# DanEngelbrecht/longtail

Measured on AMD Instinct MI355X. Metric: ingest GB/s (chunk+hash+compress), higher is better.
Workload: dtype u8/u32

## Files before the change

### include/longtail_hip.h

```cpp
#ifndef LONGTAIL_HIP_H
#define LONGTAIL_HIP_H

#include "longtail_abi.h"

#if defined(_WIN32)
#define LTHIP_EXPORT
#else
#define LTHIP_EXPORT __attribute__((visibility("default")))
#endif

#ifdef __cplusplus
extern "C" {
#endif


LTHIP_EXPORT struct Longtail_ChunkerAPI* Longtail_CreateHipChunkerAPI(void);

LTHIP_EXPORT struct Longtail_HashAPI* Longtail_CreateHipBlake3HashAPI(void);

LTHIP_EXPORT struct Longtail_HashAPI* Longtail_CreateHipBlake2HashAPI(void);

LTHIP_EXPORT struct Longtail_HashAPI* Longtail_CreateHipMeowHashAPI(void);

LTHIP_EXPORT struct Longtail_CompressionAPI* Longtail_CreateHipLZ4CompressionAPI(void);
LTHIP_EXPORT struct Longtail_CompressionAPI* Longtail_CompressionRegistry_CreateForHipLZ4(uint32_t compression_type, uint32_t* out_settings);
LTHIP_EXPORT uint32_t Longtail_GetHipLZ4DefaultQuality(void);

LTHIP_EXPORT struct Longtail_CompressionAPI* Longtail_CreateHipZStdCompressionAPI(void);
LTHIP_EXPORT struct Longtail_CompressionAPI* Longtail_CompressionRegistry_CreateForHipZstd(uint32_t compression_type, uint32_t* out_settings);

typedef void* (*Longtail_Hip_AllocFunc)(const char* context, size_t size);
typedef void (*Longtail_Hip_FreeFunc)(void* p);
LTHIP_EXPORT void Longtail_Hip_SetAllocator(Longtail_Hip_AllocFunc alloc_func, Longtail_Hip_FreeFunc free_func);

LTHIP_EXPORT int Longtail_Hip_SetDevice(int device);
LTHIP_EXPORT int Longtail_Hip_SetBlockingWaits(int on);
LTHIP_EXPORT int lthip_set_blocking_waits(int device, int on);

LTHIP_EXPORT int Longtail_Hip_GetLastError(void);

LTHIP_EXPORT uint64_t Longtail_Hip_PinnedBytes(void);
LTHIP_EXPORT void Longtail_Hip_BatchStats(uint64_t* out_batches, uint64_t* out_windows);
LTHIP_EXPORT void Longtail_Hip_CodecBatchStats(uint64_t* out_submissions, uint64_t* out_blocks);
LTHIP_EXPORT void Longtail_Hip_MemoStats(uint64_t* out_puts, uint64_t* out_hits);


typedef struct lthip_ctx lthip_ctx;
typedef struct lthip_plan lthip_plan;

#define LTHIP_STREAM_PRIVATE ((void*)(intptr_t)-1)
LTHIP_EXPORT int lthip_ctx_create(int device, void* hip_stream, lthip_ctx** out_ctx);
LTHIP_EXPORT void lthip_ctx_destroy(lthip_ctx* ctx);
LTHIP_EXPORT int lthip_ctx_sync(lthip_ctx* ctx);
LTHIP_EXPORT const char* lthip_ctx_error(const lthip_ctx* ctx);
LTHIP_EXPORT int lthip_device_count(void);
LTHIP_EXPORT const char* lthip_build_id(void);
#define LTHIP_ABI_VERSION 3
LTHIP_EXPORT int lthip_abi_version(void);

LTHIP_EXPORT int lthip_malloc_device(lthip_ctx* ctx, size_t bytes, void** out);
LTHIP_EXPORT void lthip_free_device(lthip_ctx* ctx, void* p);
LTHIP_EXPORT int lthip_malloc_pinned(lthip_ctx* ctx, size_t bytes, void** out);
LTHIP_EXPORT void lthip_free_pinned(lthip_ctx* ctx, void* p);
LTHIP_EXPORT int lthip_copy_h2d(lthip_ctx* ctx, void* d_dst, const void* h_src, size_t bytes);
LTHIP_EXPORT int lthip_copy_d2h(lthip_ctx* ctx, void* h_dst, const void* d_src, size_t bytes);
LTHIP_EXPORT int lthip_link_copy(lthip_ctx* ctx, void* dst, const void* src, size_t bytes);

enum lthip_kernel_id
{
    LTHIP_K_BUZHASH = 0,
    LTHIP_K_SELECT = 1,
    LTHIP_K_COMPACT = 2,
    LTHIP_K_B3_LEAF = 3,
    LTHIP_K_B3_PARENT = 4,
    LTHIP_K_LZ4_SEG = 5,
    LTHIP_K_LZ4_STITCH = 6,
    LTHIP_K_OTHER = 7,
    LTHIP_K_ZSTD_ENC = 8,
    LTHIP_K_GATHER = 9,
    LTHIP_K_BLAKE2S = 10,
    LTHIP_K_COUNT = 11
};
LTHIP_EXPORT int lthip_timing_enable(lthip_ctx* ctx, int on);
LTHIP_EXPORT int lthip_timing_reset(lthip_ctx* ctx);
LTHIP_EXPORT int lthip_timing_get(lthip_ctx* ctx, int kernel_id, double* out_total_ms, uint64_t* out_launches);

LTHIP_EXPORT int lthip_plan_create(lthip_ctx* ctx, uint32_t part_count, const uint64_t* part_offsets ,
                                   const uint64_t* part_sizes , uint32_t min_chunk, uint32_t avg_chunk,
                                   uint32_t max_chunk, lthip_plan** out_plan);
LTHIP_EXPORT int lthip_plan_resize_single(lthip_ctx* ctx, lthip_plan* plan, uint64_t size);
LTHIP_EXPORT int lthip_plan_reaim(lthip_ctx* ctx, lthip_plan* plan, uint32_t part_count, const uint64_t* part_offsets ,
                                  const uint64_t* part_sizes );
LTHIP_EXPORT void lthip_plan_destroy(lthip_ctx* ctx, lthip_plan* plan);
LTHIP_EXPORT uint64_t lthip_plan_chunk_capacity(const lthip_plan* plan);
LTHIP_EXPORT uint32_t lthip_plan_slices(const lthip_plan* plan);

LTHIP_EXPORT int lthip_chunk_hash(lthip_ctx* ctx, const lthip_plan* plan, const void* d_data, uint64_t* d_chunk_offsets,
                                  uint32_t* d_chunk_lens, uint64_t* d_chunk_hashes, uint32_t* d_part_first,
                                  uint64_t* out_total);

LTHIP_EXPORT int lthip_chunk_from_buffer(lthip_ctx* ctx, const void* d_data, uint64_t size, uint32_t min_chunk,
                                         uint32_t avg_chunk, uint32_t max_chunk, uint64_t* out_len);

LTHIP_EXPORT int lthip_divtest_eval(uint32_t discriminator, uint32_t hash);

LTHIP_EXPORT int lthip_hash_ranges(lthip_ctx* ctx, const void* d_data, uint64_t range_count, const uint64_t* d_offsets,
                                   const uint32_t* d_lens, uint32_t max_len ,
                                   uint64_t* d_hashes);

LTHIP_EXPORT int lthip_hash_one(lthip_ctx* ctx, const void* in, uint32_t len, uint64_t* out);

#define LTHIP_B3_STREAM_BATCH (1u << 20)
#define LTHIP_B3_STREAM_STACK_BYTES 2048u
LTHIP_EXPORT int lthip_b3_stream_batch(lthip_ctx* ctx, const void* d_data, uint64_t batch_index, void* d_stack);
LTHIP_EXPORT int lthip_b3_stream_final(lthip_ctx* ctx, const void* d_tail, uint32_t tail_len, uint64_t batch_count, const void* d_stack,
                                       uint64_t* d_out);

LTHIP_EXPORT int lthip_hash_runs_u64_bounded(lthip_ctx* ctx, const uint64_t* d_values, const uint32_t* d_first, uint32_t run_count,
                                             uint64_t total_values_bound, uint64_t run_values_bound, uint64_t* d_out);
LTHIP_EXPORT int lthip_hash_runs_u64(lthip_ctx* ctx, const uint64_t* d_values, const uint32_t* d_first, uint32_t run_count,
                                     uint64_t* d_out);

LTHIP_EXPORT int lthip_blake2s_ranges(lthip_ctx* ctx, const void* d_data, uint64_t range_count, const uint64_t* d_offsets,
                                      const uint32_t* d_lens, uint32_t max_len, uint64_t* d_hashes);
LTHIP_EXPORT int lthip_blake2s_ranges_dev(lthip_ctx* ctx, const void* d_data, uint64_t count_bound, const uint32_t* d_count,
                                          const uint64_t* d_offsets, const uint32_t* d_lens, uint32_t max_len, uint64_t* d_hashes);
LTHIP_EXPORT int lthip_blake2s_one(lthip_ctx* ctx, const void* in, uint32_t len, uint64_t* out);
LTHIP_EXPORT int lthip_blake2s_runs_u64_bounded(lthip_ctx* ctx, const uint64_t* d_values, const uint32_t* d_first, uint32_t run_count,
                                                uint64_t total_values_bound, uint64_t run_values_bound, uint64_t* d_out);
LTHIP_EXPORT int lthip_blake2s_runs_u64(lthip_ctx* ctx, const uint64_t* d_values, const uint32_t* d_first, uint32_t run_count,
                                        uint64_t* d_out);
#define LTHIP_B2S_STREAM_BATCH (1u << 20)
#define LTHIP_B2S_STREAM_STATE_BYTES 64u
LTHIP_EXPORT int lthip_b2s_stream_batch(lthip_ctx* ctx, const void* d_data, uint64_t batch_index, void* d_state);
LTHIP_EXPORT int lthip_b2s_stream_final(lthip_ctx* ctx, const void* d_tail, uint32_t tail_len, uint64_t batch_count, void* d_state,
                                        uint64_t* d_out);

#define LTHIP_MEOW_STREAM_BATCH LTHIP_B3_STREAM_BATCH
#define LTHIP_MEOW_STREAM_STATE_BYTES 136u
LTHIP_EXPORT int lthip_meow_ranges(lthip_ctx* ctx, const void* d_data, uint64_t range_count, const uint64_t* d_offsets,
                                   const uint32_t* d_lens, uint32_t max_len, uint64_t* d_hashes);
LTHIP_EXPORT int lthip_meow_ranges_dev(lthip_ctx* ctx, const void* d_data, uint64_t count_bound, const uint32_t* d_count,
                                       const uint64_t* d_offsets, const uint32_t* d_lens, uint32_t max_len, uint64_t* d_hashes);
LTHIP_EXPORT int lthip_meow_one(lthip_ctx* ctx, const void* in, uint32_t len, uint64_t* out);
LTHIP_EXPORT int lthip_meow_runs_u64_bounded(lthip_ctx* ctx, const uint64_t* d_values, const uint32_t* d_first, uint32_t run_count,
                                             uint64_t total_values_bound, uint64_t run_values_bound, uint64_t* d_out);
LTHIP_EXPORT int lthip_meow_runs_u64(lthip_ctx* ctx, const uint64_t* d_values, const uint32_t* d_first, uint32_t run_count,
                                     uint64_t* d_out);
LTHIP_EXPORT int lthip_meow_stream_batch(lthip_ctx* ctx, const void* d_data, uint64_t batch_index, void* d_state);
LTHIP_EXPORT int lthip_meow_stream_final(lthip_ctx* ctx, const void* d_tail, uint32_t tail_len, uint64_t batch_count, void* d_state,
                                         uint64_t* d_out);

LTHIP_EXPORT size_t lthip_lz4_bound(size_t size);
LTHIP_EXPORT int lthip_lz4_compress_blocks(lthip_ctx* ctx, const void* d_src, uint32_t block_count,
                                           const uint64_t* src_offsets, const uint32_t* src_sizes, void* d_dst,
                                           const uint64_t* dst_offsets, const uint32_t* dst_caps,
                                           uint32_t* d_out_sizes, int segment_log2 );
LTHIP_EXPORT int lthip_lz4_decompress_blocks(lthip_ctx* ctx, const void* d_src, uint32_t block_count,
                                             const uint64_t* src_offsets, const uint32_t* src_sizes, void* d_dst,
                                             const uint64_t* dst_offsets, const uint32_t* dst_caps,
                                             uint32_t* d_out_sizes);

LTHIP_EXPORT int lthip_pack_blocks(uint64_t chunk_count, const uint32_t* chunk_lens, uint32_t max_block_size,
                                   uint32_t max_chunks_per_block, uint64_t* block_starts, uint64_t capacity,
                                   uint64_t* out_block_count);

LTHIP_EXPORT int lthip_pack_blocks_batch(uint64_t chunk_count, const uint32_t* chunk_lens, uint64_t first_chunk,
                                         uint32_t max_block_size, uint32_t max_chunks_per_block, uint64_t max_batch_bytes,
                                         uint64_t arena_bytes, uint32_t bound_div, uint32_t bound_add,
                                         uint64_t* block_starts, uint64_t* block_sizes, uint64_t capacity,
                                         uint64_t* out_block_count, uint64_t* out_next_chunk);

LTHIP_EXPORT int lthip_gather_ranges(lthip_ctx* ctx, const void* d_src, uint64_t range_count, const uint64_t* d_src_offsets,
                                     const uint32_t* d_lens, void* d_dst, const uint64_t* d_dst_offsets);

LTHIP_EXPORT size_t lthip_zstd_bound(size_t size);
LTHIP_EXPORT int lthip_zstd_compress_blocks(lthip_ctx* ctx, const void* d_src, uint32_t block_count,
                                            const uint64_t* src_offsets, const uint32_t* src_sizes, void* d_dst,
                                            const uint64_t* dst_offsets, const uint32_t* dst_caps,
                                            uint32_t* d_out_sizes);
#define LTHIP_ZSTD_Q_DEFAULT 0
#define LTHIP_ZSTD_Q_HIGH 1
#define LTHIP_ZSTD_Q_MAX 2
LTHIP_EXPORT int lthip_zstd_quality_of_settings(uint32_t settings_id);
LTHIP_EXPORT int lthip_zstd_compress_blocks_q(lthip_ctx* ctx, const void* d_src, uint32_t block_count,
                                              const uint64_t* src_offsets, const uint32_t* src_sizes, void* d_dst,
                                              const uint64_t* dst_offsets, const uint32_t* dst_caps,
                                              uint32_t* d_out_sizes, int quality);
LTHIP_EXPORT int lthip_zstd_decompress_blocks(lthip_ctx* ctx, const void* d_src, uint32_t block_count,
                                              const uint64_t* src_offsets, const uint32_t* src_sizes, void* d_dst,
                                              const uint64_t* dst_offsets, const uint32_t* dst_caps,
                                              uint32_t* d_out_sizes);
LTHIP_EXPORT int lthip_zstd_last_decode_stats(lthip_ctx* ctx, uint32_t out[4]);
LTHIP_EXPORT void lthip_debug_reload_env(void);
LTHIP_EXPORT int lthip_debug_fail_alloc(int64_t after, int64_t count);
LTHIP_EXPORT int64_t lthip_debug_alloc_calls(int64_t* out_failed);
LTHIP_EXPORT int lthip_zstd_debug_units(lthip_ctx* ctx, uint64_t first, uint64_t count, void* h_meta, void* h_lits,
                                        void* h_recs);

LTHIP_EXPORT int lthip_dedup_first_seen(lthip_ctx* ctx, uint64_t count, const uint64_t* d_hashes,
                                        uint32_t* d_first_index, uint64_t* d_unique_count);
LTHIP_EXPORT int lthip_dedup_first_seen_range(lthip_ctx* ctx, uint64_t count, const uint64_t* d_hashes, uint64_t lookup_first,
                                              uint64_t lookup_count, uint32_t* d_first_index, uint64_t* d_unique_count);

LTHIP_EXPORT int lthip_dedup_min_ordinal(lthip_ctx* ctx, uint64_t count, const uint64_t* d_hashes, const uint32_t* d_ordinals,
                                         uint32_t* d_first_ordinal, uint64_t* d_unique_count);

LTHIP_EXPORT size_t lthip_version_index_size(uint32_t asset_count, uint64_t unique_chunk_count, uint64_t asset_chunk_index_count,
                                             uint32_t path_data_size);
LTHIP_EXPORT int lthip_build_version_index(lthip_ctx* ctx, uint32_t asset_count, const uint64_t* asset_sizes,
                                           const uint32_t* path_start_offsets, const uint16_t* permissions, const char* path_data,
                                           uint32_t path_data_size, const uint32_t* asset_chunk_counts, uint64_t chunk_total,
                                           const uint64_t* d_chunk_hashes, const uint32_t* d_chunk_lens,
                                           const uint32_t* asset_tags , uint32_t hash_identifier,
                                           uint32_t target_chunk_size, void* out, size_t out_capacity, size_t* out_size);

LTHIP_EXPORT size_t lthip_stored_block_header_size(uint32_t chunk_count);
LTHIP_EXPORT int lthip_write_stored_block_headers(lthip_ctx* ctx, uint32_t block_count, const uint64_t* block_first_chunk,
                                                  const uint64_t* d_chunk_hashes, const uint32_t* d_chunk_lens,
                                                  uint32_t hash_identifier, uint32_t tag, const uint32_t* raw_sizes,
                                                  const uint32_t* d_comp_sizes, void* d_arena, const uint64_t* image_offsets);

LTHIP_EXPORT int lthip_create_missing_content(lthip_ctx* ctx, uint64_t existing_count, const uint64_t* d_existing_hashes,
                                              uint64_t chunk_count, const uint64_t* d_chunk_hashes, const uint32_t* d_chunk_lens,
                                              const uint32_t* chunk_tags, uint32_t hash_identifier, uint32_t max_block_size,
                                              uint32_t max_chunks_per_block, void* out, size_t out_capacity, size_t* out_size);

LTHIP_EXPORT int lthip_get_existing_store_index(lthip_ctx* ctx, const void* store_index, size_t store_index_size, uint64_t chunk_count,
                                                const uint64_t* d_chunk_hashes, uint32_t min_block_usage_percent, void* out,
                                                size_t out_capacity, size_t* out_size);

enum lthip_codec
{
    LTHIP_CODEC_NONE = 0,
    LTHIP_CODEC_LZ4 = 1,
    LTHIP_CODEC_ZSTD = 2
};
typedef struct lthip_ingest lthip_ingest;
typedef struct lthip_ingest_config
{
    uint32_t target_chunk_size;
    uint32_t hash_identifier;
    uint32_t max_block_size;
    uint32_t max_chunks_per_block;
    uint32_t compression_type;
    uint32_t codec;
    uint64_t batch_bytes;
} lthip_ingest_config;
typedef struct lthip_ingest_tree
{
    uint32_t asset_count;
    const uint64_t* asset_sizes;
    const uint32_t* path_start_offsets;
    const uint16_t* permissions;
    const char* path_data;
    uint32_t path_data_size;
    const uint32_t* asset_tags;
    uint64_t job_count;
    const uint32_t* job_asset;
    const uint64_t* job_first;
    uint64_t my_job_count;
    const uint64_t* my_jobs;
} lthip_ingest_tree;
typedef struct lthip_ingest_result
{
    uint64_t struct_size;
    uint64_t chunks_all, unique_all;
    uint64_t chunks_local, unique_local;
    uint64_t blocks, raw_bytes, compressed_bytes, gathered_blocks;
    uint64_t version_index_size, store_index_size;
    uint64_t gathered_bytes;
} lthip_ingest_result;
LTHIP_EXPORT int lthip_ingest_create(lthip_ctx* ctx, const lthip_ingest_config* config, lthip_ingest** out);
LTHIP_EXPORT void lthip_ingest_destroy(lthip_ingest* ingest);
LTHIP_EXPORT int lthip_ingest_index(lthip_ingest* ingest, const lthip_ingest_tree* tree, const uint64_t* d_all_hashes,
                                    const uint32_t* d_all_lens, uint64_t all_chunks, const uint64_t* d_local_offsets,
                                    const uint32_t* d_local_part_first, uint64_t local_chunks, void* h_version_index,
                                    size_t version_index_capacity);
LTHIP_EXPORT int lthip_ingest_set_first_seen(lthip_ingest* ingest, const uint32_t* d_first_index, uint64_t unique_chunks);
LTHIP_EXPORT int lthip_ingest_write(lthip_ingest* ingest, const void* d_data, void* d_arena, uint64_t arena_bytes);
LTHIP_EXPORT int lthip_ingest_finish(lthip_ingest* ingest, void* h_store_index, size_t store_index_capacity,
                                     lthip_ingest_result* out_result);
LTHIP_EXPORT int lthip_ingest_images(const lthip_ingest* ingest, uint64_t* out_first_block, uint64_t* out_count,
                                     const uint64_t** out_offsets, const uint32_t** out_sizes);
LTHIP_EXPORT const uint32_t* lthip_ingest_compressed_sizes(const lthip_ingest* ingest);

enum lthip_partition_policy
{
    LTHIP_PARTITION_RANGE = 0,
    LTHIP_PARTITION_LPT = 1,
    LTHIP_PARTITION_MOD = 2
};
LTHIP_EXPORT uint64_t lthip_job_count(uint32_t asset_count, const uint64_t* asset_sizes, uint32_t target_chunk_size);
LTHIP_EXPORT int lthip_make_jobs(uint32_t asset_count, const uint64_t* asset_sizes, uint32_t target_chunk_size, uint64_t capacity,
                                 uint32_t* job_asset, uint64_t* job_offset , uint64_t* job_size);
LTHIP_EXPORT int lthip_partition_jobs(uint64_t job_count, const uint64_t* job_sizes, uint32_t rank_count, int policy,
                                      uint32_t* job_rank, uint64_t* rank_bytes);
LTHIP_EXPORT int lthip_exchange_layout(uint64_t job_count, const uint32_t* job_rank, uint32_t rank_count,
                                       const uint32_t* gathered_counts, uint64_t count_stride, uint64_t chunk_stride,
                                       uint64_t* job_src, uint64_t* job_dst , uint32_t* job_chunks );
LTHIP_EXPORT uint64_t lthip_exchange_ranges(uint64_t job_count, const uint64_t* job_src, const uint64_t* job_dst,
                                            const uint32_t* job_chunks, uint64_t max_piece, uint64_t capacity, uint64_t* out_src,
                                            uint64_t* out_dst, uint32_t* out_cnt);
LTHIP_EXPORT int lthip_exchange_reorder(lthip_ctx* ctx, const void* d_gathered, void* d_out, uint32_t elem_bytes,
                                        uint64_t range_count, const uint64_t* range_src, const uint64_t* range_dst,
                                        const uint32_t* range_cnt);
LTHIP_EXPORT int lthip_job_ordinals(lthip_ctx* ctx, uint64_t my_job_count, const uint32_t* local_first, const uint32_t* global_first,
                                    uint64_t local_chunks, uint32_t* d_out);

#define LTHIP_COMM_ID_BYTES 128
#define LTHIP_COMM_RCCL 1
#define LTHIP_COMM_SHM 2
typedef struct lthip_comm lthip_comm;
LTHIP_EXPORT int lthip_comm_unique_id(void* id128);
LTHIP_EXPORT int lthip_comm_create(lthip_ctx* ctx, int nranks, int rank, const void* id128, lthip_comm** out);
LTHIP_EXPORT int lthip_comm_destroy(lthip_comm* comm);
LTHIP_EXPORT const char* lthip_comm_library(const char** out_how);
LTHIP_EXPORT int lthip_comm_info(const lthip_comm* comm, int* out_nranks, int* out_rank, int* out_transport);
LTHIP_EXPORT int lthip_comm_allgather(lthip_ctx* ctx, lthip_comm* comm, const void* d_send, void* d_recv, uint64_t count,
                                      uint32_t elem_bytes);
LTHIP_EXPORT int lthip_comm_alltoallv(lthip_ctx* ctx, lthip_comm* comm, const void* d_send, const uint64_t* send_counts ,
                                      const uint64_t* send_displs , void* d_recv, const uint64_t* recv_counts ,
                                      const uint64_t* recv_displs , uint32_t elem_bytes);

LTHIP_EXPORT int lthip_synth_fill(lthip_ctx* ctx, void* d_dst, uint32_t asset_count, const uint64_t* asset_offsets ,
                                  const uint64_t* asset_sizes , const uint64_t* asset_seeds , int kind);
LTHIP_EXPORT int lthip_synth_fill_ranges(lthip_ctx* ctx, void* d_dst, uint32_t asset_count, const uint64_t* asset_offsets ,
                                         const uint64_t* asset_sizes , const uint64_t* asset_seeds ,
                                         const uint64_t* asset_skips , int kind);

#ifdef __cplusplus
}
#endif
#endif
```

### longtail_amd/csrc/k_buzhash.hip

```cpp
#include "lthip_internal.h"

#include <stdlib.h>
#include <type_traits>

namespace
{

__constant__ uint32_t c_buztab[256] = {
#include "buzhash_table.inc"
};

constexpr int RUN = 64;
constexpr int TILE = 256 * RUN;
constexpr int ROW_DW = 17;
constexpr int TAB_REP = 64;

__device__ __forceinline__ uint32_t lds_load_u32(uint32_t byte_addr)
{
#if defined(__HIP_DEVICE_COMPILE__)
    return *(const __attribute__((address_space(3))) uint32_t*)byte_addr;
#else
    (void)byte_addr;
    return 0u;
#endif
}

__device__ __forceinline__ uint32_t lds_load_u8(uint32_t byte_addr)
{
#if defined(__HIP_DEVICE_COMPILE__)
    return *(const __attribute__((address_space(3))) uint8_t*)byte_addr;
#else
    (void)byte_addr;
    return 0u;
#endif
}

__device__ __forceinline__ uint4 lds_load_u128(uint32_t byte_addr)
{
#if defined(__HIP_DEVICE_COMPILE__)
    typedef uint32_t v4 __attribute__((ext_vector_type(4)));
    const v4 q = *(const __attribute__((address_space(3))) v4*)byte_addr;
    return make_uint4(q.x, q.y, q.z, q.w);
#else
    (void)byte_addr;
    return make_uint4(0, 0, 0, 0);
#endif
}

__device__ __forceinline__ uint32_t rotl32(uint32_t x, uint32_t r) { return __builtin_amdgcn_alignbit(x, x, (32u - r) & 31u); }
__device__ __forceinline__ uint32_t rotr32(uint32_t x, uint32_t r) { return __builtin_amdgcn_alignbit(x, x, r & 31u); }

__global__ void k_tile_table(const PartDev* __restrict__ parts, uint32_t nparts, uint32_t* __restrict__ tile_part,
                             uint64_t ntiles)
{
    uint64_t t = (uint64_t)blockIdx.x * blockDim.x + threadIdx.x;
    if (t >= ntiles)
        return;
    uint32_t lo = 0, hi = nparts;
    while (hi - lo > 1)
    {
        uint32_t mid = lo + (hi - lo) / 2;
        if ((uint64_t)parts[mid].tile_base <= t)
            lo = mid;
        else
            hi = mid;
    }
    tile_part[t] = lo;
}

constexpr int WROWS = 64 + 1;
constexpr int WTILE = 64 * RUN;

#ifdef LTHIP_ABLATIONS
#include "ablations/k_buzhash_roll.inc"
#endif

#ifndef K1_MAD64
#define K1_MAD64 0
#endif
constexpr int HALO_DW = 64;

struct PrefixConsts
{
    uint32_t lane4;
    uint32_t hj;
    uint32_t halo_byte;
    uint32_t thr;
    uint32_t exact_add;
};

template <int MODE>
__device__ __forceinline__ uint64_t prefix_tile(const uint32_t (&win)[16], uint32_t hb, const PrefixConsts& pc, const DivTest& dv,
                                                int lane, uint32_t* __restrict__ halo)
{
    {
        uint32_t x = lds_load_u32((hb << 8) | pc.lane4);
        x = rotr32(x, pc.hj);
        if (lane >= 47)
            x = 0u;
        x ^= (uint32_t)__builtin_amdgcn_update_dpp(0, (int)x, 0x111, 0xf, 0xf, false);
        x ^= (uint32_t)__builtin_amdgcn_update_dpp(0, (int)x, 0x112, 0xf, 0xf, false);
        x ^= (uint32_t)__builtin_amdgcn_update_dpp(0, (int)x, 0x114, 0xf, 0xf, false);
        x ^= (uint32_t)__builtin_amdgcn_update_dpp(0, (int)x, 0x118, 0xf, 0xf, false);
        x ^= (uint32_t)__builtin_amdgcn_update_dpp(0, (int)x, 0x142, 0xa, 0xf, false);
        x ^= (uint32_t)__builtin_amdgcn_update_dpp(0, (int)x, 0x143, 0xc, 0xf, false);
        halo[pc.hj] = x;
    }

    uint32_t S[65];
#define LT_LOOKUP(j) S[j] = lds_load_u32(__builtin_amdgcn_perm(win[(j) >> 2], pc.lane4, 0x0c0c0400u | ((uint32_t)((j) & 3) << 8)))
#pragma unroll
    for (int j = 63; j >= 0; --j)
        LT_LOOKUP(j);
#undef LT_LOOKUP
    __builtin_amdgcn_sched_barrier(0);
    S[64] = 0u;
#pragma unroll
    for (int j = 63; j >= 0; --j)
        S[j] = S[j + 1] ^ ((j & 31) ? rotr32(S[j], (uint32_t)(j & 31)) : S[j]);
    __builtin_amdgcn_wave_barrier();

    uint32_t mlo = 0, mhi = 0;
    uint32_t inv_v;
    asm volatile("v_mov_b32 %0, %1" : "=v"(inv_v) : "s"(dv.inv));
#if K1_MAD64
    const uint64_t inv64 = (uint64_t)inv_v;
#endif
    typedef uint32_t u32x4 __attribute__((ext_vector_type(4)));
    u32x4 Q[16];
    auto halo_quad = [&](auto QI) __attribute__((always_inline))
    {
        constexpr int q = decltype(QI)::value;
        if constexpr (q >= 4 && q <= 15)
        {
            u32x4 v = {S[4 * q], S[4 * q + 1], S[4 * q + 2], S[4 * q + 3]};
            uint64_t save;
            asm volatile("s_mov_b64 %[sv], exec\n\ts_mov_b64 exec, %[msk]\n\t"
                         "ds_read_b128 %[r], %[ad] offset:%[o]\n\t"
                         "s_mov_b64 exec, %[sv]"
                         : [sv] "=&s"(save), [r] "+v"(v)
                         : [ad] "v"(pc.halo_byte), [msk] "s"(0x8000000000000000ull), [o] "i"(16 * q)
                         : "memory");
            Q[q] = v;
        }
    };
    auto halo_wait = [&](auto QI) __attribute__((always_inline))
    {
        constexpr int q = decltype(QI)::value;
        if constexpr (q >= 4 && q <= 15)
        {
            u32x4 v = Q[q];
            if constexpr (q >= 6)
                asm volatile("s_waitcnt lgkmcnt(2)" : "+v"(v));
            else if constexpr (q == 5)
                asm volatile("s_waitcnt lgkmcnt(1)" : "+v"(v));
            else
                asm volatile("s_waitcnt lgkmcnt(0)" : "+v"(v));
            S[4 * q] = v.x;
            S[4 * q + 1] = v.y;
            S[4 * q + 2] = v.z;
            S[4 * q + 3] = v.w;
        }
    };
    auto group = [&](auto G) __attribute__((always_inline))
    {
        constexpr int g = decltype(G)::value;
        uint32_t y[8];
#pragma unroll
        for (int half = 1; half >= 0; --half)
        {
            if (half == 1)
                halo_wait(std::integral_constant<int, 2 * g + 1 + 4>{});
            else
                halo_wait(std::integral_constant<int, 2 * g + 4>{});
#pragma unroll
            for (int ii = 3; ii >= 0; --ii)
            {
                const int i = 4 * half + ii;
                const int k = 8 * g + i;
                uint32_t w;
                if (k >= 47)
                    w = S[k - 47] ^ S[k + 1];
                else
                    w = (S[0] ^ S[k + 1]) ^ (uint32_t)__builtin_amdgcn_update_dpp(0, (int)S[(k + 17) & 63], 0x13C, 0xf, 0xf, false);
                const uint32_t h = (k & 31) ? rotl32(w, (uint32_t)(k & 31)) : w;
                if (MODE == 1)
                    y[i] = ~h & (dv.d - 1u);
                else
                {
#if K1_MAD64
                    uint64_t t, carry;
                    asm("v_mad_u64_u32 %0, %1, %2, %3, %4" : "=v"(t), "=s"(carry) : "v"(h), "s"(dv.inv), "v"(inv64));
                    y[i] = (uint32_t)t;
#else
                    y[i] = h * dv.inv + inv_v;
#endif
                }
            }
            if (half == 1)
                halo_quad(std::integral_constant<int, 2 * g + 2>{});
            else
                halo_quad(std::integral_constant<int, 2 * g + 1>{});
        }
        const uint32_t m = min(min(min(y[0], y[1]), y[2]), min(min(min(y[3], y[4]), y[5]), min(y[6], y[7])));
        if (__builtin_amdgcn_ballot_w64(m <= pc.thr) != 0ull)
        {
            asm volatile("");
#pragma unroll
            for (int i = 0; i < 8; ++i)
            {
                const int k = 8 * g + i;
                if (__builtin_amdgcn_ballot_w64(y[i] <= pc.thr) != 0ull)
                {
                    asm volatile("");
                    const bool hit = MODE == 1 ? y[i] == 0u : rotr32(y[i] + pc.exact_add, dv.k2) <= dv.qlim;
                    uint32_t hbit;
                    asm volatile("v_cndmask_b32_e64 %0, 0, 1, %1" : "=v"(hbit) : "s"(__builtin_amdgcn_ballot_w64(hit)));
                    if (k < 32)
                        mlo |= hbit << k;
                    else
                        mhi |= hbit << (k - 32);
                }
            }
        }
    };
    group(std::integral_constant<int, 7>{});
    group(std::integral_constant<int, 6>{});
    group(std::integral_constant<int, 5>{});
    group(std::integral_constant<int, 4>{});
    group(std::integral_constant<int, 3>{});
    group(std::integral_constant<int, 2>{});
    group(std::integral_constant<int, 1>{});
    group(std::integral_constant<int, 0>{});
    return ((uint64_t)mhi << 32) | mlo;
}

__device__ __forceinline__ uint64_t prefix_legal(uint64_t m, uint64_t q0, uint64_t size)
{
    if (q0 >= size)
        return 0ull;
    if (q0 < 47)
        m &= ~0ull << (47 - q0);
    const uint64_t remain = size - q0;
    if (remain < 64)
        m &= (1ull << remain) - 1ull;
    return m;
}

__device__ __forceinline__ void prefix_table_init(uint32_t* tab, int tid, int nthreads)
{
    for (int v = tid; v < 256; v += nthreads)
    {
        const uint32_t tv = c_buztab[v];
        uint4 q = make_uint4(tv, tv, tv, tv);
        uint4* dst = reinterpret_cast<uint4*>(tab + v * TAB_REP);
#pragma unroll
        for (int j = 0; j < TAB_REP / 4; ++j)
            dst[j] = q;
    }
    __syncthreads();
    if ((uint32_t)(uintptr_t)(const __attribute__((address_space(3))) uint32_t*)tab != 0u)
        __builtin_trap();
}

#ifdef LTHIP_ABLATIONS
#include "ablations/k_buzhash_prefix_regs.inc"
#endif

constexpr int DMA_BUF_B = WROWS * 64;

template <int MODE, int WAVES>
__global__ __launch_bounds__(64 * WAVES, 1) void k_buzhash_prefix_dma(const uint8_t* __restrict__ data,
                                                                       const PartDev* __restrict__ parts,
                                                                       const uint32_t* __restrict__ tile_part,
                                                                       uint32_t ntiles, DivTest dv,
                                                                       uint64_t* __restrict__ bm0,
                                                                       uint64_t* __restrict__ bm1)
{
    extern __shared__ __attribute__((aligned(16))) uint32_t smem[];
    const int tid = threadIdx.x;
    const int lane = tid & 63;
    const int wave = __builtin_amdgcn_readfirstlane(tid >> 6);
    uint32_t* buf = smem + 256 * TAB_REP + wave * ((DMA_BUF_B >> 2) + HALO_DW);
    uint32_t* halo = buf + (DMA_BUF_B >> 2);
    prefix_table_init(smem, tid, 64 * WAVES);

    const uint32_t buf_byte = __builtin_amdgcn_readfirstlane((uint32_t)(uintptr_t)(const __attribute__((address_space(3))) uint32_t*)buf);
    PrefixConsts pc;
    pc.lane4 = (uint32_t)lane * 4u;
    pc.hj = 63u - (uint32_t)lane;
    pc.halo_byte = buf_byte + DMA_BUF_B;
    pc.thr = MODE == 1 ? 0u : 0xFFFFFFFFu / (dv.d >> dv.k2);
    pc.exact_add = dv.addc - dv.inv;

    const uint32_t src_vec = 4u * ((uint32_t)lane >> 2) + (((uint32_t)lane & 3u) ^ (((uint32_t)lane >> 4) & 3u));
    const uint32_t src_off = 16u * src_vec;
    const uint32_t own_f = (((uint32_t)lane + 1u) >> 2) & 3u;
    const uint32_t own_row = buf_byte + 64u * ((uint32_t)lane + 1u);

    const uint64_t nwt = (uint64_t)ntiles * 4u;
    const uint64_t wstride = (uint64_t)gridDim.x * (uint64_t)WAVES;
    uint64_t wt = (uint64_t)blockIdx.x * (uint64_t)WAVES + (uint64_t)wave;
    if (wt >= nwt)
        return;

    const uint32_t buf_mid = buf_byte + 2048u;
    auto piece = [&](auto U, const uint8_t* mid_src) __attribute__((always_inline))
    {
        constexpr int u = decltype(U)::value;
        const uint32_t so = src_off, bm = buf_mid;
        asm volatile("s_mov_b32 m0, %[l]\n\ts_nop 0\n\t"
                     "global_load_lds_dwordx4 %[v], %[b] offset:%[o]"
                     :
                     : [v] "v"(so), [l] "s"(bm), [b] "s"(mid_src), [o] "i"(1024 * u - 2048)
                     : "memory");
    };
    auto issue = [&](const PartDev& p, uint64_t sp) __attribute__((always_inline))
    {
        const uint8_t* mid_src = data + p.off + sp - 64 + 2048;
        if (sp >= 64 && sp + (uint64_t)WTILE <= p.size)
        {
            asm volatile("s_mov_b32 m0, %[l]\n\ts_nop 0\n\t"
                         "global_load_lds_dwordx4 %[v], %[b] offset:-2048\n\t"
                         "global_load_lds_dwordx4 %[v], %[b] offset:-1024\n\t"
                         "global_load_lds_dwordx4 %[v], %[b] offset:0\n\t"
                         "global_load_lds_dwordx4 %[v], %[b] offset:1024"
                         :
                         : [v] "v"(src_off), [l] "s"(buf_mid), [b] "s"(mid_src)
                         : "memory");
            if (lane < 4)
                piece(std::integral_constant<int, 4>{}, mid_src);
        }
        else
        {
            auto edge = [&](auto U) __attribute__((always_inline))
            {
                constexpr int u = decltype(U)::value;
                const int64_t g = (int64_t)sp - 64 + 1024 * u + (int64_t)src_off;
                const bool lane_on = u < 4 || lane < 4;
                const bool whole = lane_on && g >= 0 && (uint64_t)g + 16 <= p.size;
                const bool part = lane_on && g >= 0 && (uint64_t)g < p.size && (uint64_t)g + 16 > p.size;
                if (whole)
                    piece(U, mid_src);
                if (part)
                {
                    const uint8_t* src = data + p.off;
                    uint32_t w[4] = {0, 0, 0, 0};
                    const uint32_t n = (uint32_t)(p.size - (uint64_t)g);
                    for (uint32_t bb = 0; bb < n; ++bb)
                        w[bb >> 2] |= (uint32_t)src[g + bb] << (8 * (bb & 3));
                    uint32_t* d = buf + 256 * u + 4 * lane;
                    d[0] = w[0];
                    d[1] = w[1];
                    d[2] = w[2];
                    d[3] = w[3];
                }
            };
            edge(std::integral_constant<int, 0>{});
            edge(std::integral_constant<int, 1>{});
            edge(std::integral_constant<int, 2>{});
            edge(std::integral_constant<int, 3>{});
            edge(std::integral_constant<int, 4>{});
        }
    };

    PartDev pd = parts[tile_part[wt >> 2]];
    uint64_t span = ((wt >> 2) - pd.tile_base) * (uint64_t)TILE + (wt & 3u) * (uint64_t)WTILE;
    issue(pd, span);

    uint64_t pend_m = 0, pend_summary = 0, pend_i0 = 0, pend_i1 = 0;
    bool pend = false;
    for (;;)
    {
        asm volatile("s_waitcnt vmcnt(0)" ::: "memory");
        uint32_t win[16];
#pragma unroll
        for (int c = 0; c < 4; ++c)
        {
            const uint4 q = lds_load_u128(own_row + 16u * ((uint32_t)c ^ own_f));
            win[4 * c + 0] = q.x;
            win[4 * c + 1] = q.y;
            win[4 * c + 2] = q.z;
            win[4 * c + 3] = q.w;
        }
        const uint32_t hb = lds_load_u8(buf_byte + pc.hj);
        asm volatile("s_waitcnt lgkmcnt(0)" ::: "memory");

        if (pend)
        {
            if (pend_m != 0ull)
                bm0[pend_i0 + (uint64_t)lane] = pend_m;
            if (lane == 0)
                bm1[pend_i1] = pend_summary;
        }

        const uint64_t next = wt + wstride;
        PartDev npd = pd;
        uint64_t next_span = 0;
        if (next < nwt)
        {
            npd = parts[tile_part[next >> 2]];
            next_span = ((next >> 2) - npd.tile_base) * (uint64_t)TILE + (next & 3u) * (uint64_t)WTILE;
            issue(npd, next_span);
        }

        pend_m = prefix_legal(prefix_tile<MODE>(win, hb, pc, dv, lane, halo), span + (uint64_t)lane * RUN, pd.size);
        pend_summary = __builtin_amdgcn_ballot_w64(pend_m != 0ull);
        pend_i0 = pd.bm0_base + (span >> 6);
        pend_i1 = pd.bm1_base + (span >> 12);
        pend = true;

        if (next >= nwt)
            break;
        wt = next;
        pd = npd;
        span = next_span;
    }
    if (pend_m != 0ull)
        bm0[pend_i0 + (uint64_t)lane] = pend_m;
    if (lane == 0)
        bm1[pend_i1] = pend_summary;
}

__device__ __forceinline__ uint64_t bcast64(uint64_t v, int src_lane)
{
    uint32_t lo = __builtin_amdgcn_readlane((uint32_t)v, src_lane);
    uint32_t hi = __builtin_amdgcn_readlane((uint32_t)(v >> 32), src_lane);
    return ((uint64_t)hi << 32) | lo;
}

__global__ __launch_bounds__(64) void k_select_cuts(const PartDev* __restrict__ parts, uint32_t nparts,
                                                    const uint64_t* __restrict__ bm0, const uint64_t* __restrict__ bm1,
                                                    uint32_t min_chunk, uint32_t max_chunk, uint2* __restrict__ region,
                                                    uint32_t* __restrict__ part_count)
{
    const uint32_t p = blockIdx.x;
    if (p >= nparts)
        return;
    const int lane = threadIdx.x;
    const PartDev pd = parts[p];
    const uint64_t size = pd.size;
    const uint64_t* b0 = bm0 + pd.bm0_base;
    const uint64_t* b1 = bm1 + pd.bm1_base;
    uint2* out = region + pd.region_base;

    uint64_t s = 0;
    uint32_t n = 0;
    while (s < size)
    {
        const uint64_t left = size - s;
        uint64_t len;
        if (left <= min_chunk)
            len = left;
        else
        {
            const uint64_t end = left > max_chunk ? max_chunk : left;
            len = end;
            const uint64_t qlo = s + min_chunk;
            const uint64_t qhi = s + end - 1;
            if (qlo <= qhi)
            {
                const uint64_t rlo = qlo >> 6, rhi = qhi >> 6;
                const uint64_t wlo = rlo >> 6, whi = rhi >> 6;
                bool found = false;
                for (uint64_t w0 = wlo; w0 <= whi && !found; w0 += 64)
                {
                    const uint64_t w = w0 + (uint64_t)lane;
                    uint64_t word = 0;
                    if (w <= whi)
                    {
                        word = b1[w];
                        if (w == wlo)
                            word &= ~0ull << (rlo & 63);
                        if (w == whi && (rhi & 63) != 63)
                            word &= (1ull << ((rhi & 63) + 1)) - 1ull;
                    }
                    for (;;)
                    {
                        const uint64_t any = __builtin_amdgcn_ballot_w64(word != 0ull);
                        if (any == 0ull)
                            break;
                        const int f = __builtin_ctzll(any);
                        const uint64_t fw = bcast64(word, f);
                        const int bit = __builtin_ctzll(fw);
                        const uint64_t r = ((w0 + (uint64_t)f) << 6) + (uint64_t)bit;
                        uint64_t m = b0[r];
                        if (r == rlo)
                            m &= ~0ull << (qlo & 63);
                        if (r == rhi && (qhi & 63) != 63)
                            m &= (1ull << ((qhi & 63) + 1)) - 1ull;
                        if (m != 0ull)
                        {
                            const uint64_t q = (r << 6) + (uint64_t)__builtin_ctzll(m);
                            len = q - s + 1;
                            found = true;
                            break;
                        }
                        if (lane == f)
                            word &= word - 1ull;
                    }
                }
            }
        }
        if (lane == 0)
            out[n] = make_uint2((uint32_t)s, (uint32_t)len);
        ++n;
        s += len;
    }
    if (lane == 0)
        part_count[p] = n;
}

constexpr int SCAN_THREADS = 256;
constexpr int SCAN_ITEMS = 8;
constexpr int SCAN_BLOCK = SCAN_THREADS * SCAN_ITEMS;

__device__ __forceinline__ uint32_t block_exclusive_scan(uint32_t v, uint32_t* total, uint32_t* sh )
{
    const int lane = threadIdx.x & 63, wave = threadIdx.x >> 6;
    uint32_t x = v;
#pragma unroll
    for (int o = 1; o < 64; o <<= 1)
    {
        uint32_t y = __shfl_up(x, o, 64);
        if (lane >= o)
            x += y;
    }
    if (lane == 63)
        sh[wave] = x;
    __syncthreads();
    uint32_t base = 0, tot = 0;
#pragma unroll
    for (int w = 0; w < SCAN_THREADS / 64; ++w)
    {
        uint32_t t = sh[w];
        if (w < wave)
            base += t;
        tot += t;
    }
    __syncthreads();
    *total = tot;
    return base + x - v;
}

__global__ __launch_bounds__(SCAN_THREADS) void k_scan_sums(const uint32_t* __restrict__ in, uint64_t n,
                                                            const uint32_t* __restrict__ n_dev,
                                                            uint32_t* __restrict__ sums)
{
    __shared__ uint32_t sh[8];
    if (n_dev)
        n = *n_dev < n ? *n_dev : n;
    const uint64_t base = (uint64_t)blockIdx.x * SCAN_BLOCK;
    uint32_t acc = 0;
#pragma unroll
    for (int i = 0; i < SCAN_ITEMS; ++i)
    {
        uint64_t idx = base + (uint64_t)i * SCAN_THREADS + threadIdx.x;
        if (idx < n)
            acc += in[idx];
    }
    uint32_t tot;
    block_exclusive_scan(acc, &tot, sh);
    if (threadIdx.x == 0)
        sums[blockIdx.x] = tot;
}

__global__ __launch_bounds__(SCAN_THREADS) void k_scan_spine(uint32_t* __restrict__ sums, uint32_t nblocks)
{
    __shared__ uint32_t sh[8];
    uint32_t carry = 0;
    for (uint32_t b0 = 0; b0 < nblocks; b0 += SCAN_THREADS)
    {
        uint32_t i = b0 + threadIdx.x;
        uint32_t v = i < nblocks ? sums[i] : 0;
        uint32_t tot;
        uint32_t ex = block_exclusive_scan(v, &tot, sh);
        if (i < nblocks)
            sums[i] = carry + ex;
        carry += tot;
    }
    if (threadIdx.x == 0)
        sums[nblocks] = carry;
}

__global__ __launch_bounds__(SCAN_THREADS) void k_scan_apply(const uint32_t* __restrict__ in, uint64_t n,
                                                             const uint32_t* __restrict__ n_dev,
                                                             const uint32_t* __restrict__ sums, uint32_t nblocks,
                                                             uint32_t* __restrict__ out)
{
    __shared__ uint32_t sh[8];
    if (n_dev)
        n = *n_dev < n ? *n_dev : n;
    const uint64_t base = (uint64_t)blockIdx.x * SCAN_BLOCK + (uint64_t)threadIdx.x * SCAN_ITEMS;
    uint32_t v[SCAN_ITEMS];
    uint32_t acc = 0;
#pragma unroll
    for (int i = 0; i < SCAN_ITEMS; ++i)
    {
        uint64_t idx = base + i;
        v[i] = idx < n ? in[idx] : 0;
        acc += v[i];
    }
    uint32_t tot;
    uint32_t ex = block_exclusive_scan(acc, &tot, sh) + sums[blockIdx.x];
#pragma unroll
    for (int i = 0; i < SCAN_ITEMS; ++i)
    {
        uint64_t idx = base + i;
        if (idx < n)
            out[idx] = ex;
        ex += v[i];
    }
    if (blockIdx.x == 0 && threadIdx.x == 0)
        out[n] = sums[nblocks];
}

__global__ __launch_bounds__(64) void k_compact_chunks(const PartDev* __restrict__ parts, uint32_t nparts,
                                                       const uint2* __restrict__ region,
                                                       const uint32_t* __restrict__ part_first,
                                                       uint64_t* __restrict__ chunk_offsets,
                                                       uint32_t* __restrict__ chunk_lens)
{
    const uint32_t p = blockIdx.x;
    if (p >= nparts)
        return;
    const PartDev pd = parts[p];
    const uint32_t first = part_first[p];
    const uint32_t n = part_first[p + 1] - first;
    const uint2* in = region + pd.region_base;
    for (uint32_t i = threadIdx.x; i < n; i += 64)
    {
        uint2 e = in[i];
        chunk_offsets[first + i] = pd.off + (uint64_t)e.x;
        chunk_lens[first + i] = e.y;
    }
}

__global__ __launch_bounds__(64) void k_chunk_from_buffer(const uint8_t* __restrict__ buf, uint32_t n, uint32_t min_chunk,
                                                          DivTest dv, uint64_t* __restrict__ out_len)
{
    const int lane = threadIdx.x;
    uint32_t h0 = 0;
    for (uint32_t i = 0; i < 48; ++i)
        h0 ^= rotl32(c_buztab[buf[i]], (47u - i) & 31u);
    uint32_t result = n;
    const uint32_t kmax = n - min_chunk;
    for (uint32_t k0 = 1; k0 <= kmax; k0 += 64)
    {
        const uint32_t k = k0 + (uint32_t)lane;
        bool hit = false;
        if (k <= kmax)
        {
            uint32_t h;
            if (k < 48)
            {
                h = rotl32(h0, k & 31u);
                for (uint32_t i = 1; i <= k; ++i)
                    h ^= rotl32(rotl32(c_buztab[buf[i - 1]], 16) ^ c_buztab[buf[min_chunk + i - 1]], (k - i) & 31u);
            }
            else
            {
                const uint32_t p = min_chunk + k;
                h = 0;
                for (uint32_t j = 0; j < 48; ++j)
                    h ^= rotl32(c_buztab[buf[p - 1 - j]], j & 31u);
            }
            hit = dv.pow2 ? (h & (dv.d - 1u)) == dv.d - 1u : rotr32(h * dv.inv + dv.addc, dv.k2) <= dv.qlim;
        }
        const uint64_t any = __builtin_amdgcn_ballot_w64(hit);
        if (any)
        {
            result = min_chunk + k0 + (uint32_t)__builtin_ctzll(any);
            break;
        }
    }
    if (lane == 0)
        *out_len = result;
}

}

int lthip_launch_from_buffer(lthip_ctx* ctx, const uint8_t* d_data, uint32_t n, uint32_t min_chunk, const DivTest& dv,
                             uint64_t* d_out)
{
    LaunchTimer t(ctx, LTHIP_K_OTHER);
    hipLaunchKernelGGL(k_chunk_from_buffer, dim3(1), dim3(64), 0, ctx->stream, d_data, n, min_chunk, dv, d_out);
    LTHIP_LAUNCH_CHECK(ctx);
    return 0;
}

int lthip_launch_tile_table(lthip_ctx* ctx, lthip_plan* plan)
{
    if (plan->ntiles == 0)
        return 0;
    LaunchTimer t(ctx, LTHIP_K_OTHER);
    const uint32_t blocks = (uint32_t)div_up_u64(plan->ntiles, 256);
    hipLaunchKernelGGL(k_tile_table, dim3(blocks), dim3(256), 0, ctx->stream, plan->d_parts, plan->nparts,
                       plan->d_tile_part, plan->ntiles);
    LTHIP_LAUNCH_CHECK(ctx);
    return 0;
}

#ifdef LTHIP_ABLATIONS
constexpr bool K1_HAS_REG_FLAVOUR = true;
#else
constexpr bool K1_HAS_REG_FLAVOUR = false;
#endif

template <int WAVES, bool DMA>
static int launch_buzhash_prefix(lthip_ctx* ctx, const lthip_plan* plan, const uint8_t* d_data, uint64_t* bm0, uint64_t* bm1)
{
    static_assert(DMA || K1_HAS_REG_FLAVOUR, "the register-staged flavour is compiled by the ablation build only");
    constexpr size_t per_wave = DMA ? (DMA_BUF_B >> 2) + HALO_DW : WROWS * ROW_DW + HALO_DW;
    static_assert(sizeof(uint32_t) * (256 * TAB_REP + WAVES * per_wave) <= 160 * 1024, "LDS budget: one workgroup per CU");
    const size_t lds = sizeof(uint32_t) * (256 * TAB_REP + WAVES * per_wave);
#ifdef LTHIP_ABLATIONS
    auto k0 = DMA ? &k_buzhash_prefix_dma<0, WAVES> : &k_buzhash_prefix<0, WAVES>;
    auto k1 = DMA ? &k_buzhash_prefix_dma<1, WAVES> : &k_buzhash_prefix<1, WAVES>;
#else
    auto k0 = &k_buzhash_prefix_dma<0, WAVES>;
    auto k1 = &k_buzhash_prefix_dma<1, WAVES>;
#endif
    static bool granted[64] = {};
    if (ctx->device < 0 || ctx->device >= 64 || !granted[ctx->device])
    {
        LTHIP_CHECK(ctx, hipFuncSetAttribute(reinterpret_cast<const void*>(k0), hipFuncAttributeMaxDynamicSharedMemorySize, (int)lds));
        LTHIP_CHECK(ctx, hipFuncSetAttribute(reinterpret_cast<const void*>(k1), hipFuncAttributeMaxDynamicSharedMemorySize, (int)lds));
        if (ctx->device >= 0 && ctx->device < 64)
            granted[ctx->device] = true;
    }
    int ncu = 256;
    (void)hipDeviceGetAttribute(&ncu, hipDeviceAttributeMultiprocessorCount, ctx->device);
    uint32_t grid = (uint32_t)ncu;
    if ((uint64_t)grid * WAVES > plan->ntiles * 4u)
        grid = (uint32_t)div_up_u64(plan->ntiles * 4u, WAVES);
    LaunchTimer t(ctx, LTHIP_K_BUZHASH);
    hipLaunchKernelGGL(plan->div.pow2 ? k1 : k0, dim3(grid), dim3(64 * WAVES), lds, ctx->stream, d_data, plan->d_parts,
                       plan->d_tile_part, (uint32_t)plan->ntiles, plan->div, bm0, bm1);
    LTHIP_LAUNCH_CHECK(ctx);
    return 0;
}

#ifdef LTHIP_ABLATIONS
static int k1_flavour()
{
    static std::atomic<int> f{-1};
    static std::atomic<uint32_t> seen{0};
    const uint32_t gen = g_lthip_env_gen;
    if (seen.load(std::memory_order_acquire) != gen)
    {
        const char* e = getenv("LTHIP_K1");
        f.store(!e ? 0 : !strcmp(e, "roll") ? 4 : !strcmp(e, "prefix12") ? 3 : !strcmp(e, "prefix16") ? 2 : !strcmp(e, "dma12") ? 1 : 0,
                std::memory_order_relaxed);
        seen.store(gen, std::memory_order_release);
    }
    return f.load(std::memory_order_relaxed);
}

static int launch_buzhash_roll(lthip_ctx* ctx, const lthip_plan* plan, const uint8_t* d_data, uint64_t* bm0, uint64_t* bm1)
{
    static_assert(sizeof(uint32_t) * (256 * TAB_REP + K1_WAVES * WROWS * ROW_DW) <= 160 * 1024, "LDS budget: one workgroup per CU");
    const size_t lds = sizeof(uint32_t) * (256 * TAB_REP + K1_WAVES * WROWS * ROW_DW);
    if (!ctx->k1_lds_enabled)
    {
        LTHIP_CHECK(ctx, hipFuncSetAttribute(reinterpret_cast<const void*>(&k_buzhash_candidates<0>), hipFuncAttributeMaxDynamicSharedMemorySize, (int)lds));
        LTHIP_CHECK(ctx, hipFuncSetAttribute(reinterpret_cast<const void*>(&k_buzhash_candidates<1>), hipFuncAttributeMaxDynamicSharedMemorySize, (int)lds));
        ctx->k1_lds_enabled = true;
    }
    int ncu = 256;
    (void)hipDeviceGetAttribute(&ncu, hipDeviceAttributeMultiprocessorCount, ctx->device);
    uint32_t grid = (uint32_t)ncu;
    if ((uint64_t)grid * K1_WAVES > plan->ntiles * 4u)
        grid = (uint32_t)div_up_u64(plan->ntiles * 4u, K1_WAVES);
    LaunchTimer t(ctx, LTHIP_K_BUZHASH);
    if (plan->div.pow2)
        hipLaunchKernelGGL(k_buzhash_candidates<1>, dim3(grid), dim3(K1_THREADS), lds, ctx->stream, d_data, plan->d_parts,
                           plan->d_tile_part, (uint32_t)plan->ntiles, plan->div, bm0, bm1);
    else
        hipLaunchKernelGGL(k_buzhash_candidates<0>, dim3(grid), dim3(K1_THREADS), lds, ctx->stream, d_data, plan->d_parts,
                           plan->d_tile_part, (uint32_t)plan->ntiles, plan->div, bm0, bm1);
    LTHIP_LAUNCH_CHECK(ctx);
    return 0;
}
#endif

int lthip_launch_buzhash(lthip_ctx* ctx, const lthip_plan* plan, const uint8_t* d_data, uint64_t* bm0, uint64_t* bm1)
{
    if (plan->ntiles == 0)
        return 0;
#ifdef LTHIP_ABLATIONS
    const int flavour = k1_flavour();
    if (flavour == 1)
        return launch_buzhash_prefix<12, true>(ctx, plan, d_data, bm0, bm1);
    if (flavour == 2)
        return launch_buzhash_prefix<16, false>(ctx, plan, d_data, bm0, bm1);
    if (flavour == 3)
        return launch_buzhash_prefix<12, false>(ctx, plan, d_data, bm0, bm1);
    if (flavour == 4)
        return launch_buzhash_roll(ctx, plan, d_data, bm0, bm1);
#endif
    return launch_buzhash_prefix<16, true>(ctx, plan, d_data, bm0, bm1);
}

int lthip_launch_select(lthip_ctx* ctx, const lthip_plan* plan, const uint64_t* bm0, const uint64_t* bm1, uint2* region,
                        uint32_t* part_count)
{
    LaunchTimer t(ctx, LTHIP_K_SELECT);
    hipLaunchKernelGGL(k_select_cuts, dim3(plan->nparts), dim3(64), 0, ctx->stream, plan->d_parts, plan->nparts, bm0, bm1,
                       plan->min_chunk, plan->max_chunk, region, part_count);
    LTHIP_LAUNCH_CHECK(ctx);
    return 0;
}

int lthip_exclusive_scan_u32(lthip_ctx* ctx, const uint32_t* d_in, uint32_t* d_out, uint64_t n_bound,
                             const uint32_t* d_n, int kid)
{
    const uint64_t nblocks64 = n_bound ? div_up_u64(n_bound, SCAN_BLOCK) : 1;
    if (nblocks64 > 0x7FFFFFFFull)
        return lthip_fail(ctx, EINVAL, "scan", "too many elements");
    const uint32_t nblocks = (uint32_t)nblocks64;
    void* tmp;
    int err = lthip_scratch(ctx, S_SCAN_TMP, ((size_t)nblocks + 1) * 4, &tmp);
    if (err)
        return err;
    uint32_t* sums = (uint32_t*)tmp;
    LaunchTimer t(ctx, kid);
    hipLaunchKernelGGL(k_scan_sums, dim3(nblocks), dim3(SCAN_THREADS), 0, ctx->stream, d_in, n_bound, d_n, sums);
    hipLaunchKernelGGL(k_scan_spine, dim3(1), dim3(SCAN_THREADS), 0, ctx->stream, sums, nblocks);
    hipLaunchKernelGGL(k_scan_apply, dim3(nblocks), dim3(SCAN_THREADS), 0, ctx->stream, d_in, n_bound, d_n, sums, nblocks,
                       d_out);
    LTHIP_LAUNCH_CHECK(ctx);
    return 0;
}

int lthip_launch_compact(lthip_ctx* ctx, const lthip_plan* plan, const uint2* region, const uint32_t* part_count,
                         uint32_t* d_part_first, uint64_t* d_chunk_offsets, uint32_t* d_chunk_lens)
{
    int err = lthip_exclusive_scan_u32(ctx, part_count, d_part_first, plan->nparts, nullptr, LTHIP_K_COMPACT);
    if (err || plan->nparts == 0)
        return err;
    LaunchTimer t(ctx, LTHIP_K_COMPACT);
    hipLaunchKernelGGL(k_compact_chunks, dim3(plan->nparts), dim3(64), 0, ctx->stream, plan->d_parts, plan->nparts, region,
                       (const uint32_t*)d_part_first, d_chunk_offsets, d_chunk_lens);
    LTHIP_LAUNCH_CHECK(ctx);
    return 0;
}
```

### longtail_amd/csrc/lthip_ctx.hip

```cpp
#include "lthip_internal.h"

#include <stdlib.h>

int lthip_fail(lthip_ctx* ctx, int code, const char* what, const char* detail)
{
    if (ctx)
        snprintf(ctx->err, sizeof ctx->err, "%s: %s", what ? what : "?", detail ? detail : "");
    return code;
}

int lthip_scratch(lthip_ctx* ctx, int slot, size_t bytes, void** out)
{
    if (bytes == 0)
        bytes = 256;
    if (ctx->scratch_cap[slot] < bytes)
    {
        if (ctx->scratch[slot])
        {
            LTHIP_CHECK(ctx, lthip_stream_wait(ctx));
            LTHIP_CHECK(ctx, hipFree(ctx->scratch[slot]));
            ctx->scratch[slot] = nullptr;
            ctx->scratch_cap[slot] = 0;
        }
        size_t cap = bytes + bytes / 8 + 4096;
        LTHIP_CHECK(ctx, lthip_hip_malloc(&ctx->scratch[slot], cap));
        ctx->scratch_cap[slot] = cap;
    }
    *out = ctx->scratch[slot];
    return 0;
}

volatile uint32_t g_lthip_env_gen = 1;
extern "C" void lthip_debug_reload_env(void) { g_lthip_env_gen = g_lthip_env_gen + 1u; }

#ifdef LTHIP_ABLATIONS
namespace
{
std::atomic<int64_t> g_alloc_calls{0};
std::atomic<int64_t> g_fail_first{INT64_MAX};
std::atomic<int64_t> g_fail_last{INT64_MAX};
std::atomic<int64_t> g_alloc_failed{0};
bool inject_failure()
{
    const int64_t n = g_alloc_calls.fetch_add(1, std::memory_order_relaxed) + 1;
    if (n < g_fail_first.load(std::memory_order_relaxed) || n > g_fail_last.load(std::memory_order_relaxed))
        return false;
    g_alloc_failed.fetch_add(1, std::memory_order_relaxed);
    return true;
}
}
hipError_t lthip_hip_malloc(void** p, size_t bytes)
{
    if (inject_failure())
    {
        *p = nullptr;
        return hipErrorOutOfMemory;
    }
    return hipMalloc(p, bytes);
}
hipError_t lthip_hip_host_malloc(void** p, size_t bytes, unsigned flags)
{
    if (inject_failure())
    {
        *p = nullptr;
        return hipErrorOutOfMemory;
    }
    return hipHostMalloc(p, bytes, flags);
}
extern "C" int lthip_debug_fail_alloc(int64_t after, int64_t count)
{
    if (after < 0 || count <= 0)
    {
        g_fail_first = INT64_MAX;
        g_fail_last = INT64_MAX;
        return 0;
    }
    const int64_t now = g_alloc_calls.load();
    g_fail_last = INT64_MAX;
    g_fail_first = now + after + 1;
    g_fail_last = count > INT64_MAX - (now + after) ? INT64_MAX : now + after + count;
    return 0;
}
extern "C" int64_t lthip_debug_alloc_calls(int64_t* out_failed)
{
    if (out_failed)
        *out_failed = g_alloc_failed.load();
    return g_alloc_calls.load();
}
#else
extern "C" int lthip_debug_fail_alloc(int64_t, int64_t) { return ENOTSUP; }
extern "C" int64_t lthip_debug_alloc_calls(int64_t* out_failed)
{
    if (out_failed)
        *out_failed = 0;
    return -1;
}
#endif

extern "C" int lthip_device_count(void)
{
    int n = 0;
    if (hipGetDeviceCount(&n) != hipSuccess)
        return 0;
    return n;
}

extern "C" int lthip_ctx_create(int device, void* hip_stream, lthip_ctx** out_ctx)
{
    if (!out_ctx)
        return EINVAL;
    *out_ctx = nullptr;
    int n = 0;
    if (hipGetDeviceCount(&n) != hipSuccess || n <= 0)
        return ENODEV;
    if (device < 0 || device >= n)
        return EINVAL;
    if (hipSetDevice(device) != hipSuccess)
        return EIO;
    lthip_ctx* ctx = new (std::nothrow) lthip_ctx();
    if (!ctx)
        return ENOMEM;
    ctx->device = device;
    ctx->slice_ctx = nullptr;
    ctx->err[0] = 0;
    ctx->timing = false;
    memset(ctx->scratch, 0, sizeof ctx->scratch);
    memset(ctx->stage, 0, sizeof ctx->stage);
    memset(ctx->stage_small, 0, sizeof ctx->stage_small);
    ctx->stage_next = ctx->stage_small_next = 0;
    ctx->k1_lds_enabled = false;
    ctx->z_last_retry = nullptr;
    ctx->z_last_payloads = 0;
    ctx->z_last_foreign_blocks = 0;
    memset(ctx->k5_lds_enabled, 0, sizeof ctx->k5_lds_enabled);
    memset(ctx->scratch_cap, 0, sizeof ctx->scratch_cap);
    memset(ctx->total_ms, 0, sizeof ctx->total_ms);
    memset(ctx->launches, 0, sizeof ctx->launches);
    if (hip_stream != LTHIP_STREAM_PRIVATE)
    {
        ctx->stream = (hipStream_t)hip_stream;
        ctx->own_stream = false;
    }
    else
    {
        if (hipStreamCreateWithFlags(&ctx->stream, hipStreamNonBlocking) != hipSuccess)
        {
            delete ctx;
            return EIO;
        }
        ctx->own_stream = true;
    }
    *out_ctx = ctx;
    return 0;
}

hipError_t lthip_stream_wait(lthip_ctx* ctx) { return hipStreamSynchronize(ctx->stream); }

extern "C" int lthip_set_blocking_waits(int device, int on)
{
    int n = 0;
    if (hipGetDeviceCount(&n) != hipSuccess || device < 0 || device >= n)
        return ENODEV;
    int prev = 0;
    (void)hipGetDevice(&prev);
    if (hipSetDevice(device) != hipSuccess)
        return EIO;
    const hipError_t e = hipSetDeviceFlags(on ? hipDeviceScheduleBlockingSync : hipDeviceScheduleAuto);
    (void)hipSetDevice(prev);
    return e == hipSuccess ? 0 : EIO;
}

extern "C" void lthip_ctx_destroy(lthip_ctx* ctx)
{
    if (!ctx)
        return;
    (void)hipSetDevice(ctx->device);
    (void)hipStreamSynchronize(ctx->stream);
    if (ctx->slice_ctx)
        lthip_ctx_destroy(ctx->slice_ctx);
    for (auto& r : ctx->pending)
    {
        (void)hipEventDestroy(r.a);
        (void)hipEventDestroy(r.b);
    }
    for (auto e : ctx->free_events)
        (void)hipEventDestroy(e);
    for (auto e : ctx->sync_events)
        (void)hipEventDestroy(e);
    if (ctx->stream2)
    {
        (void)hipStreamSynchronize(ctx->stream2);
        (void)hipStreamDestroy(ctx->stream2);
    }
    for (int i = 0; i < S_COUNT; ++i)
        if (ctx->scratch[i])
            (void)hipFree(ctx->scratch[i]);
    for (auto& st : ctx->stage)
    {
        if (st.done)
            (void)hipEventDestroy(st.done);
        if (st.p)
            (void)hipHostFree(st.p);
    }
    for (auto& st : ctx->stage_small)
    {
        if (st.done)
            (void)hipEventDestroy(st.done);
        if (st.p)
            (void)hipHostFree(st.p);
    }
    if (ctx->own_stream)
        (void)hipStreamDestroy(ctx->stream);
    delete ctx;
}

extern "C" int lthip_ctx_sync(lthip_ctx* ctx)
{
    if (!ctx)
        return EINVAL;
    LTHIP_CHECK(ctx, lthip_stream_wait(ctx));
    return 0;
}

extern "C" const char* lthip_ctx_error(const lthip_ctx* ctx) { return ctx ? ctx->err : "no context"; }

extern "C" int lthip_malloc_device(lthip_ctx* ctx, size_t bytes, void** out)
{
    if (!ctx || !out)
        return EINVAL;
    LTHIP_CHECK(ctx, hipSetDevice(ctx->device));
    LTHIP_CHECK(ctx, lthip_hip_malloc(out, bytes ? bytes : 16));
    return 0;
}

extern "C" void lthip_free_device(lthip_ctx* ctx, void* p)
{
    if (!p)
        return;
    if (ctx)
    {
        (void)hipSetDevice(ctx->device);
        (void)lthip_stream_wait(ctx);
    }
    (void)hipFree(p);
}

extern "C" int lthip_malloc_pinned(lthip_ctx* ctx, size_t bytes, void** out)
{
    if (!ctx || !out)
        return EINVAL;
    LTHIP_CHECK(ctx, hipSetDevice(ctx->device));
    LTHIP_CHECK(ctx, lthip_hip_host_malloc(out, bytes ? bytes : 16, hipHostMallocDefault));
    return 0;
}

extern "C" void lthip_free_pinned(lthip_ctx* ctx, void* p)
{
    if (!p)
        return;
    if (ctx)
    {
        (void)hipSetDevice(ctx->device);
        (void)lthip_stream_wait(ctx);
    }
    (void)hipHostFree(p);
}

extern "C" int lthip_copy_h2d(lthip_ctx* ctx, void* d_dst, const void* h_src, size_t bytes)
{
    if (!ctx || (bytes && (!d_dst || !h_src)))
        return EINVAL;
    if (bytes == 0)
        return 0;
    LTHIP_CHECK(ctx, hipSetDevice(ctx->device));
    LTHIP_CHECK(ctx, hipMemcpyAsync(d_dst, h_src, bytes, hipMemcpyHostToDevice, ctx->stream));
    return 0;
}

extern "C" int lthip_copy_d2h(lthip_ctx* ctx, void* h_dst, const void* d_src, size_t bytes)
{
    if (!ctx || (bytes && (!h_dst || !d_src)))
        return EINVAL;
    if (bytes == 0)
        return 0;
    LTHIP_CHECK(ctx, hipSetDevice(ctx->device));
    LTHIP_CHECK(ctx, hipMemcpyAsync(h_dst, d_src, bytes, hipMemcpyDeviceToHost, ctx->stream));
    return 0;
}

static hipEvent_t take_event(lthip_ctx* ctx)
{
    if (!ctx->free_events.empty())
    {
        hipEvent_t e = ctx->free_events.back();
        ctx->free_events.pop_back();
        return e;
    }
    hipEvent_t e = nullptr;
    (void)hipEventCreate(&e);
    return e;
}

LaunchTimer::LaunchTimer(lthip_ctx* c, int kid, hipStream_t s) : ctx(c), on(c->timing), stream(s ? s : c->stream)
{
    if (on)
    {
        rec.kid = kid;
        rec.a = take_event(ctx);
        rec.b = take_event(ctx);
        (void)hipEventRecord(rec.a, stream);
    }
}

int lthip_second_stream(lthip_ctx* ctx, hipStream_t* out)
{
    if (!ctx->stream2)
        LTHIP_CHECK(ctx, hipStreamCreateWithFlags(&ctx->stream2, hipStreamNonBlocking));
    *out = ctx->stream2;
    return 0;
}

int lthip_stage_upload(lthip_ctx* ctx, void* d_dst, const void* h_src, size_t bytes, hipStream_t stream)
{
    if (bytes == 0)
        return 0;
    const bool small = bytes <= LTHIP_STAGE_SMALL;
    LTHIP_ABLATION_ENV(env_slots, "LTHIP_STAGE_SLOTS");
    const size_t nsmall = env_slots.get() > 0 && env_slots.get() < 64 ? (size_t)env_slots.get() : sizeof(ctx->stage_small) / sizeof(ctx->stage_small[0]);
    lthip_ctx::Stage& st = small ? ctx->stage_small[ctx->stage_small_next++ % nsmall]
                                 : ctx->stage[ctx->stage_next++ % (sizeof(ctx->stage) / sizeof(ctx->stage[0]))];
    if (st.used)
        LTHIP_CHECK(ctx, hipEventSynchronize(st.done));
    if (st.cap < bytes)
    {
        if (st.p)
            LTHIP_CHECK(ctx, hipHostFree(st.p));
        st.p = nullptr;
        st.cap = 0;
        const size_t want = small ? LTHIP_STAGE_SMALL : bytes + bytes / 2 + 4096;
        LTHIP_CHECK(ctx, lthip_hip_host_malloc(&st.p, want, hipHostMallocDefault));
        st.cap = want;
    }
    if (!st.done)
        LTHIP_CHECK(ctx, hipEventCreateWithFlags(&st.done, hipEventDisableTiming));
    memcpy(st.p, h_src, bytes);
    LTHIP_CHECK(ctx, hipMemcpyAsync(d_dst, st.p, bytes, hipMemcpyHostToDevice, stream));
    LTHIP_CHECK(ctx, hipEventRecord(st.done, stream));
    st.used = true;
    return 0;
}

hipEvent_t lthip_sync_event(lthip_ctx* ctx)
{
    if (ctx->sync_events.size() < 16)
    {
        hipEvent_t e = nullptr;
        (void)hipEventCreateWithFlags(&e, hipEventDisableTiming);
        ctx->sync_events.push_back(e);
        return e;
    }
    return ctx->sync_events[ctx->sync_next++ % ctx->sync_events.size()];
}

LaunchTimer::~LaunchTimer()
{
    if (on)
    {
        (void)hipEventRecord(rec.b, stream);
        ctx->pending.push_back(rec);
    }
}

static int timing_collect(lthip_ctx* ctx)
{
    if (ctx->pending.empty())
        return 0;
    LTHIP_CHECK(ctx, lthip_stream_wait(ctx));
    for (auto& r : ctx->pending)
    {
        float ms = 0.f;
        if (hipEventElapsedTime(&ms, r.a, r.b) == hipSuccess)
        {
            ctx->total_ms[r.kid] += (double)ms;
            ctx->launches[r.kid] += 1;
        }
        ctx->free_events.push_back(r.a);
        ctx->free_events.push_back(r.b);
    }
    ctx->pending.clear();
    return 0;
}

extern "C" int lthip_timing_enable(lthip_ctx* ctx, int on)
{
    if (!ctx)
        return EINVAL;
    int err = timing_collect(ctx);
    ctx->timing = on != 0;
    if (ctx->slice_ctx)
        (void)lthip_timing_enable(ctx->slice_ctx, on);
    return err;
}

extern "C" int lthip_timing_reset(lthip_ctx* ctx)
{
    if (!ctx)
        return EINVAL;
    int err = timing_collect(ctx);
    memset(ctx->total_ms, 0, sizeof ctx->total_ms);
    memset(ctx->launches, 0, sizeof ctx->launches);
    if (ctx->slice_ctx)
        (void)lthip_timing_reset(ctx->slice_ctx);
    return err;
}

extern "C" int lthip_timing_get(lthip_ctx* ctx, int kernel_id, double* out_total_ms, uint64_t* out_launches)
{
    if (!ctx || kernel_id < 0 || kernel_id >= LTHIP_K_COUNT)
        return EINVAL;
    int err = timing_collect(ctx);
    double ms = ctx->total_ms[kernel_id];
    uint64_t n = ctx->launches[kernel_id];
    if (ctx->slice_ctx)
    {
        double ms2 = 0;
        uint64_t n2 = 0;
        if (lthip_timing_get(ctx->slice_ctx, kernel_id, &ms2, &n2) == 0)
        {
            ms += ms2;
            n += n2;
        }
    }
    if (out_total_ms)
        *out_total_ms = ms;
    if (out_launches)
        *out_launches = n;
    return err;
}

static uint32_t discriminator_from_avg(uint32_t avg)
{
    double a = (double)avg;
    return (uint32_t)(a / (-1.42888852e-7 * a + 1.33237515));
}

static DivTest make_div_test(uint32_t d)
{
    DivTest t;
    memset(&t, 0, sizeof t);
    t.d = d;
    if (d == 0)
        return t;
    uint32_t k2 = 0, dodd = d;
    while ((dodd & 1u) == 0)
    {
        dodd >>= 1;
        ++k2;
    }
    uint32_t inv = dodd;
    for (int i = 0; i < 5; ++i)
        inv *= 2u - dodd * inv;
    t.inv = inv;
    t.k2 = k2;
    t.addc = inv - (1u << k2);
    t.qlim = (uint32_t)(0xFFFFFFFFull / d) - 1u;
    t.pow2 = dodd == 1u;
    return t;
}

extern "C" int lthip_pack_blocks(uint64_t chunk_count, const uint32_t* chunk_lens, uint32_t max_block_size,
                                 uint32_t max_chunks_per_block, uint64_t* block_starts, uint64_t capacity, uint64_t* out_block_count)
{
    if (!out_block_count || (chunk_count && (!chunk_lens || !block_starts)) || max_block_size == 0 || max_chunks_per_block == 0)
        return EINVAL;
    const uint64_t limit = (uint64_t)max_block_size + max_block_size / 10;
    uint64_t i = 0, nb = 0;
    while (i < chunk_count)
    {
        if (nb + 1 >= capacity)
            return ENOMEM;
        block_starts[nb++] = i;
        uint64_t size = chunk_lens[i];
        uint32_t n = 1;
        while (i + 1 < chunk_count && n < max_chunks_per_block && size + chunk_lens[i + 1] <= limit)
        {
            size += chunk_lens[i + 1];
            ++n;
            ++i;
        }
        ++i;
    }
    if (capacity == 0)
        return ENOMEM;
    block_starts[nb] = chunk_count;
    *out_block_count = nb;
    return 0;
}

extern "C" int lthip_pack_blocks_batch(uint64_t chunk_count, const uint32_t* chunk_lens, uint64_t first_chunk,
                                       uint32_t max_block_size, uint32_t max_chunks_per_block, uint64_t max_batch_bytes,
                                       uint64_t arena_bytes, uint32_t bound_div, uint32_t bound_add, uint64_t* block_starts,
                                       uint64_t* block_sizes, uint64_t capacity, uint64_t* out_block_count,
                                       uint64_t* out_next_chunk)
{
    if (!out_block_count || !out_next_chunk || !block_starts || !block_sizes || (chunk_count && !chunk_lens) ||
        max_block_size == 0 || max_chunks_per_block == 0 || bound_div == 0 || capacity < 2 || first_chunk > chunk_count)
        return EINVAL;
    const uint64_t limit = (uint64_t)max_block_size + max_block_size / 10;
    uint64_t i = first_chunk, nb = 0, bytes = 0, arena = 0;
    while (i < chunk_count && nb + 1 < capacity)
    {
        const uint64_t start = i;
        uint64_t size = chunk_lens[i];
        uint32_t n = 1;
        while (i + 1 < chunk_count && n < max_chunks_per_block && size + chunk_lens[i + 1] <= limit)
        {
            size += chunk_lens[i + 1];
            ++n;
            ++i;
        }
        ++i;
        const uint64_t bound = (size + size / bound_div + bound_add + 63u) & ~(uint64_t)63u;
        if (nb && (bytes + size > max_batch_bytes || arena + bound > arena_bytes))
        {
            i = start;
            break;
        }
        block_starts[nb] = start;
        block_sizes[nb] = size;
        ++nb;
        bytes += size;
        arena += bound;
    }
    block_starts[nb] = i;
    *out_block_count = nb;
    *out_next_chunk = i;
    return 0;
}

extern "C" int lthip_divtest_eval(uint32_t discriminator, uint32_t hash)
{
    if (discriminator == 0)
        return 0;
    const DivTest t = make_div_test(discriminator);
    if (t.pow2)
        return (hash & (t.d - 1u)) == t.d - 1u;
    const uint32_t m = hash * t.inv + t.addc;
    const uint32_t r = t.k2 ? ((m >> t.k2) | (m << (32u - t.k2))) : m;
    return r <= t.qlim;
}

static uint32_t plan_slice_points(uint32_t part_count, const uint64_t* part_sizes, uint32_t want, uint32_t* first)
{
    if (part_count < 2 || want < 2)
        return 0;
    uint64_t total = 0;
    for (uint32_t p = 0; p < part_count; ++p)
        total += part_sizes[p];
    if (total < LTHIP_SLICE_MIN_BYTES)
        return 0;
    uint32_t S = want > part_count ? part_count : want;
    while (S > 2 && total / S < LTHIP_SLICE_MIN_BYTES / 2)
        --S;
    uint64_t acc = 0;
    uint32_t p = 0;
    first[0] = 0;
    for (uint32_t k = 1; k < S; ++k)
    {
        const uint64_t goal = total / S * k;
        while (p < part_count - (S - k) && acc + part_sizes[p] / 2 < goal)
            acc += part_sizes[p++];
        if (p <= first[k - 1])
        {
            acc += part_sizes[p];
            ++p;
        }
        first[k] = p;
    }
    first[S] = part_count;
    return S;
}

static int plan_layout(lthip_ctx* ctx, const char* what, uint32_t min_chunk, uint32_t part_count, const uint64_t* part_offsets,
                       const uint64_t* part_sizes, PartDev* parts, PlanExtents& x)
{
    memset(&x, 0, sizeof x);
    x.nparts = part_count;
    for (uint32_t p = 0; p < part_count; ++p)
    {
        const uint64_t sz = part_sizes[p];
        if ((part_offsets[p] & 15u) != 0 || sz > 0xFFFFFFFFull)
            return lthip_fail(ctx, EINVAL, what, "part offsets must be 16-byte aligned, sizes < 4 GiB");
        PartDev& pd = parts[p];
        memset(&pd, 0, sizeof pd);
        pd.off = part_offsets[p];
        pd.size = sz;
        pd.bm0_base = x.bm0_words;
        pd.bm1_base = x.bm1_words;
        pd.region_base = x.chunk_cap;
        pd.tile_base = (uint32_t)x.ntiles;
        const uint64_t cap = sz ? sz / min_chunk + 1 : 0;
        pd.region_cap = (uint32_t)cap;
        const uint64_t t = div_up_u64(sz, 16384);
        x.ntiles += t;
        x.bm0_words += t * 256;
        x.bm1_words += t * 4;
        x.chunk_cap += cap;
        x.total_bytes += sz;
        x.leaf_cap += div_up_u64(sz, 1024) + cap;
    }
    return 0;
}

static int plan_create_impl(lthip_ctx* ctx, uint32_t part_count, const uint64_t* part_offsets, const uint64_t* part_sizes,
                            uint32_t min_chunk, uint32_t avg_chunk, uint32_t max_chunk, lthip_plan** out_plan)
{
    if (!ctx || !out_plan || (part_count && (!part_offsets || !part_sizes)))
        return EINVAL;
    *out_plan = nullptr;
    if (min_chunk < 48 || min_chunk > avg_chunk || avg_chunk > max_chunk)
        return lthip_fail(ctx, EINVAL, "lthip_plan_create", "need 48 <= min <= avg <= max");
    uint32_t d = discriminator_from_avg(avg_chunk);
    if (d == 0)
        return lthip_fail(ctx, EINVAL, "lthip_plan_create", "discriminator is zero");
    LTHIP_CHECK(ctx, hipSetDevice(ctx->device));
    std::vector<PartDev> parts(part_count);
    PlanExtents x;
    int err = plan_layout(ctx, "lthip_plan_create", min_chunk, part_count, part_offsets, part_sizes, parts.data(), x);
    if (err)
        return err;
    if (x.ntiles > 0xFFFFFFF0ull)
        return lthip_fail(ctx, EINVAL, "lthip_plan_create", "batch too large");

    lthip_plan* plan = new (std::nothrow) lthip_plan();
    if (!plan)
        return ENOMEM;
    memset(plan, 0, sizeof *plan);
    static_cast<PlanExtents&>(*plan) = x;
    plan->device = ctx->device;
    plan->min_chunk = min_chunk;
    plan->avg_chunk = avg_chunk;
    plan->max_chunk = max_chunk;
    plan->div = make_div_test(d);
    plan->capacity_bytes = x.total_bytes;
    plan->cap_parts = part_count ? part_count : 1;
    plan->cap_tiles = x.ntiles ? x.ntiles : 1;

    hipError_t e = lthip_hip_malloc((void**)&plan->d_parts, sizeof(PartDev) * plan->cap_parts);
    if (e == hipSuccess)
        e = lthip_hip_malloc((void**)&plan->d_tile_part, sizeof(uint32_t) * plan->cap_tiles);
    if (e == hipSuccess && part_count)
        e = hipMemcpyAsync(plan->d_parts, parts.data(), sizeof(PartDev) * part_count, hipMemcpyHostToDevice, ctx->stream);
    if (e == hipSuccess)
        e = lthip_stream_wait(ctx);
    if (e != hipSuccess)
    {
        lthip_plan_destroy(ctx, plan);
        return lthip_fail(ctx, e == hipErrorOutOfMemory ? ENOMEM : EIO, "lthip_plan_create", hipGetErrorString(e));
    }
    if ((err = lthip_launch_tile_table(ctx, plan)))
    {
        lthip_plan_destroy(ctx, plan);
        return err;
    }
    *out_plan = plan;
    return 0;
}

static int plan_aim(lthip_ctx* ctx, lthip_plan* plan, const PlanExtents& x, const PartDev* parts)
{
    static_cast<PlanExtents&>(*plan) = x;
    const int err = lthip_stage_upload(ctx, plan->d_parts, parts, sizeof(PartDev) * x.nparts, ctx->stream);
    return err ? err : lthip_launch_tile_table(ctx, plan);
}

static void plan_aim_slices(lthip_ctx* ctx, lthip_plan* plan, uint32_t want, const uint64_t* part_offsets, const uint64_t* part_sizes)
{
    plan->sliced = false;
    uint32_t first[9];
    const uint32_t S = plan_slice_points(plan->nparts, part_sizes, want, first);
    if (S == 0 || (plan->nslices && S != plan->nslices))
        return;
    bool ok = true;
    if (!plan->nslices)
        for (uint32_t k = 0; k < S && ok; ++k)
            ok = plan_create_impl(ctx, first[k + 1] - first[k], part_offsets + first[k], part_sizes + first[k], plan->min_chunk,
                                  plan->avg_chunk, plan->max_chunk, &plan->slice[k]) == 0;
    else
    {
        std::vector<PartDev> parts(plan->nparts);
        PlanExtents x[8];
        for (uint32_t k = 0; k < S && ok; ++k)
        {
            const uint32_t n = first[k + 1] - first[k];
            ok = plan_layout(ctx, "lthip_plan_reaim", plan->min_chunk, n, part_offsets + first[k], part_sizes + first[k], &parts[first[k]],
                             x[k]) == 0 &&
                 n <= plan->slice[k]->cap_parts && x[k].ntiles <= plan->slice[k]->cap_tiles;
        }
        for (uint32_t k = 0; k < S && ok; ++k)
            ok = plan_aim(ctx, plan->slice[k], x[k], &parts[first[k]]) == 0;
    }
    if (!ok)
    {
        if (!plan->nslices)
            for (uint32_t k = 0; k < S; ++k)
            {
                lthip_plan_destroy(ctx, plan->slice[k]);
                plan->slice[k] = nullptr;
            }
        ctx->err[0] = 0;
        return;
    }
    memcpy(plan->slice_first, first, sizeof(uint32_t) * (S + 1));
    plan->nslices = S;
    plan->sliced = true;
}

extern "C" int lthip_plan_create(lthip_ctx* ctx, uint32_t part_count, const uint64_t* part_offsets,
                                 const uint64_t* part_sizes, uint32_t min_chunk, uint32_t avg_chunk, uint32_t max_chunk,
                                 lthip_plan** out_plan)
{
    int err = plan_create_impl(ctx, part_count, part_offsets, part_sizes, min_chunk, avg_chunk, max_chunk, out_plan);
    if (err)
        return err;
    int want = LTHIP_SLICES;
    LTHIP_ABLATION_ENV(env_slices, "LTHIP_SLICES");
    if (env_slices.get() > 0)
        want = env_slices.get() > 8 ? 8 : env_slices.get();
    plan_aim_slices(ctx, *out_plan, (uint32_t)want, part_offsets, part_sizes);
    return 0;
}

extern "C" int lthip_plan_resize_single(lthip_ctx* ctx, lthip_plan* plan, uint64_t size)
{
    if (!ctx || !plan || plan->nparts != 1)
        return EINVAL;
    if (size > plan->capacity_bytes)
        return lthip_fail(ctx, EINVAL, "lthip_plan_resize_single", "size above the capacity the plan was created with");
    LTHIP_CHECK(ctx, hipSetDevice(ctx->device));
    const uint64_t off = 0;
    PartDev pd;
    PlanExtents x;
    const int err = plan_layout(ctx, "lthip_plan_resize_single", plan->min_chunk, 1, &off, &size, &pd, x);
    if (err)
        return err;
    static_cast<PlanExtents&>(*plan) = x;
    return lthip_stage_upload(ctx, plan->d_parts, &pd, sizeof pd, ctx->stream);
}

extern "C" int lthip_plan_reaim(lthip_ctx* ctx, lthip_plan* plan, uint32_t part_count, const uint64_t* part_offsets,
                                const uint64_t* part_sizes)
{
    if (!ctx || !plan || (part_count && (!part_offsets || !part_sizes)))
        return EINVAL;
    if (part_count == 0 || part_count > plan->cap_parts)
        return lthip_fail(ctx, EINVAL, "lthip_plan_reaim", "part count outside 1 .. the count the plan was created with");
    LTHIP_CHECK(ctx, hipSetDevice(ctx->device));
    {
        std::vector<PartDev> parts(part_count);
        PlanExtents x;
        int err = plan_layout(ctx, "lthip_plan_reaim", plan->min_chunk, part_count, part_offsets, part_sizes, parts.data(), x);
        if (err)
            return err;
        if (x.ntiles > plan->cap_tiles)
            return lthip_fail(ctx, EINVAL, "lthip_plan_reaim", "more 16 KiB tiles than the plan was created with");
        if ((err = plan_aim(ctx, plan, x, parts.data())))
            return err;
    }
    if (plan->nslices)
        plan_aim_slices(ctx, plan, plan->nslices, part_offsets, part_sizes);
    return 0;
}

extern "C" void lthip_plan_destroy(lthip_ctx* ctx, lthip_plan* plan)
{
    if (!plan)
        return;
    (void)hipSetDevice(plan->device);
    if (ctx)
        (void)lthip_stream_wait(ctx);
    else
        (void)hipDeviceSynchronize();
    if (plan->d_parts)
        (void)hipFree(plan->d_parts);
    if (plan->d_tile_part)
        (void)hipFree(plan->d_tile_part);
    for (uint32_t k = 0; k < 8; ++k)
        lthip_plan_destroy(ctx, plan->slice[k]);
    delete plan;
}

extern "C" uint64_t lthip_plan_chunk_capacity(const lthip_plan* plan) { return plan ? plan->chunk_cap : 0; }
extern "C" uint32_t lthip_plan_slices(const lthip_plan* plan) { return plan && plan->sliced ? plan->nslices : 1u; }

static int chunk_bitmaps(lthip_ctx* ctx, const lthip_plan* plan, uint64_t** bm0, uint64_t** bm1)
{
    const int err = lthip_scratch(ctx, S_BM0, plan->bm0_words * 8, (void**)bm0);
    return err ? err : lthip_scratch(ctx, S_BM1, plan->bm1_words * 8, (void**)bm1);
}

static int chunk_scan(lthip_ctx* ctx, const lthip_plan* plan, const void* d_data, uint64_t* bm0, uint64_t* bm1)
{
    return plan->nparts ? lthip_launch_buzhash(ctx, plan, (const uint8_t*)d_data, bm0, bm1) : 0;
}

static int chunk_cut_hash(lthip_ctx* ctx, const lthip_plan* plan, const void* d_data, const uint64_t* bm0, const uint64_t* bm1,
                          uint64_t* d_offsets, uint32_t* d_lens, uint64_t* d_hashes, uint32_t* d_part_first)
{
    void *region, *pcount;
    int err;
    if ((err = lthip_scratch(ctx, S_REGION, plan->chunk_cap * sizeof(uint2), &region)) ||
        (err = lthip_scratch(ctx, S_PART_COUNT, ((size_t)plan->nparts + 1) * 4, &pcount)))
        return err;
    if (plan->nparts && (err = lthip_launch_select(ctx, plan, bm0, bm1, (uint2*)region, (uint32_t*)pcount)))
        return err;
    if ((err = lthip_launch_compact(ctx, plan, (const uint2*)region, (const uint32_t*)pcount, d_part_first, d_offsets, d_lens)))
        return err;
    return d_hashes ? lthip_launch_blake3(ctx, (const uint8_t*)d_data, d_offsets, d_lens, d_part_first + plan->nparts, plan->chunk_cap,
                                          plan->leaf_cap, plan->max_chunk, d_hashes)
                    : 0;
}

__global__ void k_slice_join(const uint64_t* __restrict__ b_off, const uint32_t* __restrict__ b_len, const uint64_t* __restrict__ b_hash,
                             const uint32_t* __restrict__ b_first, uint32_t nparts_b, uint32_t* __restrict__ part_first ,
                             uint64_t* __restrict__ offs, uint32_t* __restrict__ lens, uint64_t* __restrict__ hashes)
{
    const uint32_t base = part_first[0], total_b = b_first[nparts_b];
    const uint64_t i = (uint64_t)blockIdx.x * blockDim.x + threadIdx.x;
    if (i < total_b)
    {
        offs[base + i] = b_off[i];
        lens[base + i] = b_len[i];
        hashes[base + i] = b_hash[i];
    }
    if (i >= 1 && i <= nparts_b)
        part_first[i] = b_first[i] + base;
}

static int chunk_hash_sliced(lthip_ctx* ctx, const lthip_plan* plan, const void* d_data, uint64_t* d_chunk_offsets, uint32_t* d_chunk_lens, uint64_t* d_chunk_hashes, uint32_t* d_part_first,
                             bool* taken)
{
    *taken = false;
    if (!plan->sliced || !d_chunk_hashes)
        return 0;
    if (!ctx->slice_ctx && lthip_ctx_create(ctx->device, LTHIP_STREAM_PRIVATE, &ctx->slice_ctx) != 0)
        return 0;
    lthip_ctx* c2 = ctx->slice_ctx;
    const uint32_t S = plan->nslices;
    uint64_t cap_rest = 0, parts_rest = 0;
    for (uint32_t k = 1; k < S; ++k)
    {
        cap_rest += plan->slice[k]->chunk_cap + 1;
        parts_rest += (uint64_t)plan->slice[k]->nparts + 1;
    }
    void *x_off, *x_len, *x_hash, *x_first;
    uint64_t *bm0, *bm1;
    if (lthip_scratch(ctx, S_SLICE_OFFS, cap_rest * 8, &x_off) || lthip_scratch(ctx, S_SLICE_LENS, cap_rest * 4, &x_len) ||
        lthip_scratch(ctx, S_SLICE_HASH, cap_rest * 8, &x_hash) || lthip_scratch(ctx, S_SLICE_FIRST, parts_rest * 4, &x_first) ||
        chunk_bitmaps(ctx, plan, &bm0, &bm1))
    {
        ctx->err[0] = 0;
        return 0;
    }
    *taken = true;
    c2->timing = ctx->timing;

    int err = 0;
    uint64_t co = 0, po = 0;
    uint64_t *offs_k[8], *hash_k[8];
    uint32_t *lens_k[8], *first_k[8];
    for (uint32_t k = 0; k < S && !err; ++k)
    {
        const lthip_plan* pk = plan->slice[k];
        offs_k[k] = k ? (uint64_t*)x_off + co : d_chunk_offsets;
        lens_k[k] = k ? (uint32_t*)x_len + co : d_chunk_lens;
        hash_k[k] = k ? (uint64_t*)x_hash + co : d_chunk_hashes;
        first_k[k] = k ? (uint32_t*)x_first + po : d_part_first;
        co += k ? pk->chunk_cap + 1 : 0;
        po += k ? (uint64_t)pk->nparts + 1 : 0;
        if ((err = chunk_scan(ctx, pk, d_data, bm0, bm1)))
            break;
        hipEvent_t scanned = lthip_sync_event(ctx);
        hipError_t e = hipEventRecord(scanned, ctx->stream);
        if (e == hipSuccess)
            e = hipStreamWaitEvent(c2->stream, scanned, 0);
        if (e != hipSuccess)
            err = lthip_fail(ctx, EIO, "lthip_chunk_hash (the wait of the second stream for a scan)", hipGetErrorString(e));
        else if ((err = chunk_cut_hash(c2, pk, d_data, bm0, bm1, offs_k[k], lens_k[k], hash_k[k], first_k[k])))
            (void)lthip_fail(ctx, err, "lthip_chunk_hash (a slice on the second stream)", c2->err);
        bm0 += pk->bm0_words;
        bm1 += pk->bm1_words;
    }
    hipEvent_t hashed = lthip_sync_event(ctx);
    hipError_t e = hipEventRecord(hashed, c2->stream);
    if (e == hipSuccess)
        e = hipStreamWaitEvent(ctx->stream, hashed, 0);
    if (e != hipSuccess)
    {
        (void)hipStreamSynchronize(c2->stream);
        if (!err)
            err = lthip_fail(ctx, EIO, "lthip_chunk_hash (the join of the second stream)", hipGetErrorString(e));
    }
    if (!err)
    {
        LaunchTimer t(ctx, LTHIP_K_COMPACT);
        for (uint32_t k = 1; k < S; ++k)
        {
            const lthip_plan* pk = plan->slice[k];
            const uint64_t n = pk->chunk_cap > (uint64_t)pk->nparts + 1 ? pk->chunk_cap : (uint64_t)pk->nparts + 1;
            hipLaunchKernelGGL(k_slice_join, dim3((uint32_t)div_up_u64(n, 256)), dim3(256), 0, ctx->stream, (const uint64_t*)offs_k[k], (const uint32_t*)lens_k[k],
                               (const uint64_t*)hash_k[k], (const uint32_t*)first_k[k], pk->nparts, d_part_first + plan->slice_first[k], d_chunk_offsets,
                               d_chunk_lens, d_chunk_hashes);
        }
        if ((e = hipGetLastError()) != hipSuccess)
            err = lthip_fail(ctx, EIO, "kernel launch", hipGetErrorString(e));
    }
    return err;
}

extern "C" int lthip_chunk_hash(lthip_ctx* ctx, const lthip_plan* plan, const void* d_data, uint64_t* d_chunk_offsets,
                                uint32_t* d_chunk_lens, uint64_t* d_chunk_hashes, uint32_t* d_part_first,
                                uint64_t* out_total)
{
    if (!ctx || !plan || !d_chunk_offsets || !d_chunk_lens || !d_part_first || (plan->total_bytes && !d_data))
        return EINVAL;
    LTHIP_CHECK(ctx, hipSetDevice(ctx->device));
    bool sliced;
    int err = chunk_hash_sliced(ctx, plan, d_data, d_chunk_offsets, d_chunk_lens, d_chunk_hashes, d_part_first, &sliced);
    uint64_t *bm0, *bm1;
    if (!sliced && !(err = chunk_bitmaps(ctx, plan, &bm0, &bm1)) && !(err = chunk_scan(ctx, plan, d_data, bm0, bm1)))
        err = chunk_cut_hash(ctx, plan, d_data, bm0, bm1, d_chunk_offsets, d_chunk_lens, d_chunk_hashes, d_part_first);
    if (err)
        return err;
    if (out_total)
    {
        uint32_t total = 0;
        LTHIP_CHECK(ctx, hipMemcpyAsync(&total, d_part_first + plan->nparts, 4, hipMemcpyDeviceToHost, ctx->stream));
        LTHIP_CHECK(ctx, lthip_stream_wait(ctx));
        *out_total = total;
    }
    return 0;
}

extern "C" int lthip_chunk_from_buffer(lthip_ctx* ctx, const void* d_data, uint64_t size, uint32_t min_chunk,
                                       uint32_t avg_chunk, uint32_t max_chunk, uint64_t* out_len)
{
    if (!ctx || !d_data || !out_len || size == 0)
        return EINVAL;
    if (min_chunk < 48 || min_chunk > avg_chunk || avg_chunk > max_chunk)
        return lthip_fail(ctx, EINVAL, "lthip_chunk_from_buffer", "need 48 <= min <= avg <= max");
    if (size <= min_chunk)
    {
        *out_len = size;
        return 0;
    }
    const uint32_t d = discriminator_from_avg(avg_chunk);
    if (d == 0)
        return lthip_fail(ctx, EINVAL, "lthip_chunk_from_buffer", "discriminator is zero");
    LTHIP_CHECK(ctx, hipSetDevice(ctx->device));
    void* d_out;
    int err = lthip_scratch(ctx, S_MISC, 64, &d_out);
    if (err)
        return err;
    const uint32_t n = (uint32_t)(size > max_chunk ? max_chunk : size);
    if ((err = lthip_launch_from_buffer(ctx, (const uint8_t*)d_data, n, min_chunk, make_div_test(d), (uint64_t*)d_out)))
        return err;
    uint64_t len = 0;
    LTHIP_CHECK(ctx, hipMemcpyAsync(&len, d_out, 8, hipMemcpyDeviceToHost, ctx->stream));
    LTHIP_CHECK(ctx, lthip_stream_wait(ctx));
    *out_len = len;
    return 0;
}
```

### longtail_amd/csrc/lthip_internal.h

```cpp
#pragma once

#include <hip/hip_runtime.h>

#include <errno.h>
#include <stdint.h>
#include <stdio.h>
#include <stdlib.h>
#include <string.h>

#include <atomic>
#include <vector>

#include "../../include/longtail_hip.h"

struct PartDev
{
    uint64_t off;
    uint64_t size;
    uint64_t bm0_base;
    uint64_t bm1_base;
    uint64_t region_base;
    uint32_t tile_base;
    uint32_t region_cap;
};

struct DivTest
{
    uint32_t d;
    uint32_t inv;
    uint32_t addc;
    uint32_t k2;
    uint32_t qlim;
    uint32_t pow2;
};

struct PlanExtents
{
    uint32_t nparts;
    uint64_t total_bytes;
    uint64_t ntiles;
    uint64_t chunk_cap;
    uint64_t bm0_words;
    uint64_t bm1_words;
    uint64_t leaf_cap;
};

struct lthip_plan : PlanExtents
{
    int device;
    uint32_t min_chunk, avg_chunk, max_chunk;
    DivTest div;
    uint64_t capacity_bytes;
    uint32_t cap_parts;
    uint64_t cap_tiles;
    PartDev* d_parts;
    uint32_t* d_tile_part;
    lthip_plan* slice[8];
    uint32_t slice_first[9];
    uint32_t nslices;
    bool sliced;
};
constexpr uint64_t LTHIP_SLICE_MIN_BYTES = 1ull << 30;
#ifndef LTHIP_SLICES
#define LTHIP_SLICES 2
#endif

enum ScratchSlot
{
    S_BM0 = 0,
    S_BM1,
    S_REGION,
    S_PART_COUNT,
    S_LEAF_COUNT,
    S_LEAF_PREFIX,
    S_SCAN_TMP,
    S_CV,
    S_LZ4_SEGS,
    S_LZ4_META,
    S_LZ4_STREAM,
    S_LZ4_BLOCKS,
    S_TABLES,
    S_TABLES2,
    S_MISC,
    S_Z_LITS,
    S_Z_RECS,
    S_Z_ENC,
    S_Z_WORK,
    S_Z_SUB,
    S_LZ4_WORKLIST,
    S_LZ4_LANE_RECS,
    S_LZ4_CLASSIFY,
    S_B3_WINDOWS,
    S_Z_FR,
    S_Z_ORG,
    S_Z_PERM,
    S_XCHG,
    S_XCHG2,
    S_SLICE_OFFS,
    S_SLICE_LENS,
    S_SLICE_HASH,
    S_SLICE_FIRST,
    S_LEN_CLASS_ORDER,
    S_COUNT
};

struct TimingRec
{
    int kid;
    hipEvent_t a, b;
};

struct lthip_ctx
{
    int device;
    hipStream_t stream;
    bool own_stream;
    lthip_ctx* slice_ctx;
    hipStream_t stream2;
    std::vector<hipEvent_t> sync_events;
    size_t sync_next;
    char err[320];
    struct Stage
    {
        void* p;
        size_t cap;
        hipEvent_t done;
        bool used;
    };
    Stage stage[8], stage_small[64];
    size_t stage_small_next;
    size_t stage_next;
    bool k1_lds_enabled;
    bool k5_lds_enabled[2][2];
    bool k5h_lds_enabled[2];
    void* scratch[S_COUNT];
    size_t scratch_cap[S_COUNT];
    bool timing;
    std::vector<TimingRec> pending;
    std::vector<hipEvent_t> free_events;
    const uint32_t* z_last_retry;
    uint32_t z_last_payloads, z_last_foreign_blocks;
    double total_ms[LTHIP_K_COUNT];
    uint64_t launches[LTHIP_K_COUNT];
};

int lthip_fail(lthip_ctx* ctx, int code, const char* what, const char* detail);
hipError_t lthip_stream_wait(lthip_ctx* ctx);

extern volatile uint32_t g_lthip_env_gen;
struct LthipEnvInt
{
    const char* name;
    std::atomic<int> value{-1};
    std::atomic<uint32_t> seen{0};
    explicit LthipEnvInt(const char* n) : name(n) {}
    int get()
    {
        const uint32_t gen = g_lthip_env_gen;
        if (seen.load(std::memory_order_acquire) != gen)
        {
            const char* e = getenv(name);
            value.store(e ? atoi(e) : -1, std::memory_order_relaxed);
            seen.store(gen, std::memory_order_release);
        }
        return value.load(std::memory_order_relaxed);
    }
};
#ifdef LTHIP_ABLATIONS
#define LTHIP_ABLATION_ENV(var, name) static LthipEnvInt var{name}
#else
struct LthipEnvOff
{
    constexpr int get() const { return -1; }
};
#define LTHIP_ABLATION_ENV(var, name) constexpr LthipEnvOff var{}
#endif
#ifdef LTHIP_ABLATIONS
hipError_t lthip_hip_malloc(void** p, size_t bytes);
hipError_t lthip_hip_host_malloc(void** p, size_t bytes, unsigned flags);
#else
static inline hipError_t lthip_hip_malloc(void** p, size_t bytes) { return hipMalloc(p, bytes); }
static inline hipError_t lthip_hip_host_malloc(void** p, size_t bytes, unsigned flags) { return hipHostMalloc(p, bytes, flags); }
#endif
int lthip_scratch(lthip_ctx* ctx, int slot, size_t bytes, void** out);
int lthip_second_stream(lthip_ctx* ctx, hipStream_t* out);
hipEvent_t lthip_sync_event(lthip_ctx* ctx);
constexpr uint32_t LTHIP_ZSTD_CHAIN = 8;
uint64_t lthip_codec_batch_bytes();
uint64_t lthip_origin_budget_mib();
constexpr size_t LTHIP_STAGE_SMALL = 64u << 10;
int lthip_stage_upload(lthip_ctx* ctx, void* d_dst, const void* h_src, size_t bytes, hipStream_t stream);

#define LTHIP_CHECK(ctx, expr)                                                          \
    do                                                                                  \
    {                                                                                   \
        hipError_t e__ = (expr);                                                        \
        if (e__ != hipSuccess)                                                          \
            return lthip_fail((ctx), e__ == hipErrorOutOfMemory ? ENOMEM : EIO, #expr, hipGetErrorString(e__)); \
    } while (0)

struct LaunchTimer
{
    lthip_ctx* ctx;
    TimingRec rec;
    bool on;
    hipStream_t stream;
    LaunchTimer(lthip_ctx* c, int kid, hipStream_t s = nullptr);
    ~LaunchTimer();
};

#define LTHIP_LAUNCH_CHECK(ctx)                                                          \
    do                                                                                   \
    {                                                                                    \
        hipError_t e__ = hipGetLastError();                                              \
        if (e__ != hipSuccess)                                                           \
            return lthip_fail((ctx), EIO, "kernel launch", hipGetErrorString(e__));      \
    } while (0)

int lthip_launch_tile_table(lthip_ctx* ctx, lthip_plan* plan);
int lthip_launch_buzhash(lthip_ctx* ctx, const lthip_plan* plan, const uint8_t* d_data, uint64_t* bm0, uint64_t* bm1);
int lthip_launch_select(lthip_ctx* ctx, const lthip_plan* plan, const uint64_t* bm0, const uint64_t* bm1, uint2* region,
                        uint32_t* part_count);
int lthip_launch_compact(lthip_ctx* ctx, const lthip_plan* plan, const uint2* region, const uint32_t* part_count,
                         uint32_t* d_part_first, uint64_t* d_chunk_offsets, uint32_t* d_chunk_lens);
int lthip_exclusive_scan_u32(lthip_ctx* ctx, const uint32_t* d_in, uint32_t* d_out, uint64_t n_bound, const uint32_t* d_n,
                             int kid);
int lthip_launch_blake3(lthip_ctx* ctx, const uint8_t* d_data, const uint64_t* d_offsets, const uint32_t* d_lens,
                        const uint32_t* d_count, uint64_t count_bound, uint64_t leaf_bound, uint64_t max_len,
                        uint64_t* d_hashes);

int lthip_hash_ranges_known(lthip_ctx* ctx, const void* d_data, uint64_t range_count, const uint64_t* d_offsets, const uint32_t* d_lens,
                            uint32_t max_len, uint64_t leaf_total, uint64_t* d_hashes);

int lthip_launch_blake3_stream_batch(lthip_ctx* ctx, const void* d_data, uint32_t leaf0, uint32_t* d_stack, uint32_t depth_in, uint32_t merges);
int lthip_launch_blake3_stream_final(lthip_ctx* ctx, const void* d_tail, uint32_t tail_len, uint32_t leaf0, const uint32_t* d_stack,
                                     uint32_t depth, uint64_t* d_out);
int lthip_launch_blake3_one(lthip_ctx* ctx, const void* in, uint32_t len, uint64_t* out);

struct ChainHash
{
    int (*ranges)(lthip_ctx* ctx, const uint8_t* d_data, const uint64_t* d_offsets, const uint32_t* d_lens, const uint32_t* d_count,
                  uint64_t count_bound, uint64_t* d_hashes);
    int (*one)(lthip_ctx* ctx, const void* in, uint32_t len, uint64_t* out);
    int (*stream)(lthip_ctx* ctx, const void* d_data, uint32_t len, uint32_t* d_state, int first, int final, uint64_t* d_out);
    uint32_t stream_batch;
};
const ChainHash* lthip_chain_blake2s();
const ChainHash* lthip_chain_meow();
int lthip_len_class_order(lthip_ctx* ctx, const uint32_t* d_lens, const uint32_t* d_count, uint64_t count_bound, uint32_t unit_shift,
                          uint32_t long_class, const uint32_t** order, const uint32_t** n_long);

constexpr uint32_t LTHIP_HASH_BLAKE3 = 0x626c6b33u;
constexpr uint32_t LTHIP_HASH_BLAKE2 = 0x626c6b32u;
constexpr uint32_t LTHIP_HASH_MEOW = 0x6d656f77u;
const ChainHash* lthip_chain_hash(uint32_t hash_identifier);
int lthip_hash_ranges_by_id(lthip_ctx* ctx, uint32_t hash_identifier, const void* d_data, uint64_t range_count, const uint64_t* d_offsets,
                            const uint32_t* d_lens, uint32_t max_len, uint64_t leaf_total, uint64_t* d_hashes);

int lthip_launch_from_buffer(lthip_ctx* ctx, const uint8_t* d_data, uint32_t n, uint32_t min_chunk, const DivTest& dv,
                             uint64_t* d_out);

int lthip_launch_lz_sequences(lthip_ctx* ctx, const void* d_src, uint32_t block_count, const uint64_t* src_offsets,
                              const uint32_t* src_sizes, void* d_dst, const uint64_t* dst_offsets, const uint32_t* dst_caps,
                              uint8_t** d_lits, uint64_t** d_recs, void** d_meta, uint32_t* unit_base, uint64_t* total_units, int quality);

static inline uint64_t div_up_u64(uint64_t a, uint64_t b) { return (a + b - 1) / b; }
```

### longtail_amd/lib.py

```python
from __future__ import annotations

import ctypes as C
import errno
import os
from pathlib import Path
from typing import Optional, Sequence

import numpy as np

_LIB_PATH = Path(os.environ["LTHIP_LIB_PATH"]) if os.environ.get("LTHIP_LIB_PATH") else Path(__file__).resolve().parent / "liblongtail_hip.so"

KERNEL_IDS = {
    "buzhash": 0,
    "select": 1,
    "compact": 2,
    "blake3_leaf": 3,
    "blake3_parent": 4,
    "lz4_segments": 5,
    "lz4_stitch": 6,
    "other": 7,
    "zstd_encode": 8,
    "gather": 9,
}
BLAKE2S_KERNEL_ID = 10
HASH_BLAKE3 = 0x626C6B33
HASH_BLAKE2 = 0x626C6B32
B2S_STREAM_BATCH = 1 << 20
B2S_STREAM_STATE_BYTES = 64
HASH_MEOW = 0x6D656F77
MEOW_STREAM_BATCH = 1 << 20
MEOW_STREAM_STATE_BYTES = 136


class LongtailHipError(RuntimeError):
    def __init__(self, code: int, what: str, detail: str = ""):
        self.code = code
        super().__init__(f"{what}: errno {code} ({errno.errorcode.get(code, '?')}) {detail}")


def _u64arr(a: Sequence[int]) -> np.ndarray:
    return np.ascontiguousarray(np.asarray(a, dtype=np.uint64))


def _u32arr(a: Sequence[int]) -> np.ndarray:
    return np.ascontiguousarray(np.asarray(a, dtype=np.uint32))


ABI_VERSION = 3


class HipLib:

    def __init__(self, path: Optional[os.PathLike] = None):
        p = Path(path) if path else _LIB_PATH
        if not p.exists():
            raise FileNotFoundError(
                f"{p} is missing: run `python -c 'import __graft_entry__ as g; g.build()'` or `make` first "
                "(there is no CPU fallback)"
            )
        self.path = p
        try:
            import torch
        except ImportError:
            pass
        self.dll = C.CDLL(str(p))
        d = self.dll
        vp, u64, u32, i32, sz = C.c_void_p, C.c_uint64, C.c_uint32, C.c_int, C.c_size_t
        P = C.POINTER

        def sig(name, res, args):
            f = getattr(d, name)
            f.restype = res
            f.argtypes = args
            return f

        sig("Longtail_CreateHipChunkerAPI", vp, [])
        sig("Longtail_CreateHipBlake3HashAPI", vp, [])
        sig("Longtail_CreateHipBlake2HashAPI", vp, [])
        sig("Longtail_CreateHipMeowHashAPI", vp, [])
        sig("Longtail_CreateHipLZ4CompressionAPI", vp, [])
        sig("Longtail_CompressionRegistry_CreateForHipLZ4", vp, [u32, P(u32)])
        sig("Longtail_GetHipLZ4DefaultQuality", u32, [])
        sig("Longtail_CreateHipZStdCompressionAPI", vp, [])
        sig("Longtail_CompressionRegistry_CreateForHipZstd", vp, [u32, P(u32)])
        sig("Longtail_Hip_SetAllocator", None, [vp, vp])
        sig("Longtail_Hip_SetDevice", i32, [i32])
        sig("Longtail_Hip_GetLastError", i32, [])
        sig("Longtail_Hip_PinnedBytes", u64, [])
        sig("Longtail_Hip_BatchStats", None, [vp, vp])
        sig("Longtail_Hip_MemoStats", None, [vp, vp])
        sig("lthip_ctx_create", i32, [i32, vp, P(vp)])
        sig("lthip_ctx_destroy", None, [vp])
        sig("lthip_ctx_sync", i32, [vp])
        sig("lthip_ctx_error", C.c_char_p, [vp])
        sig("lthip_device_count", i32, [])
        sig("lthip_build_id", C.c_char_p, [])
        sig("lthip_abi_version", i32, [])
        if d.lthip_abi_version() != ABI_VERSION:
            raise RuntimeError(f"{p}: binary interface version {d.lthip_abi_version()}, this binding was written for {ABI_VERSION} "
                               "(include/longtail_hip.h LTHIP_ABI_VERSION): rebuild the library")
        sig("lthip_malloc_device", i32, [vp, sz, P(vp)])
        sig("lthip_free_device", None, [vp, vp])
        sig("lthip_malloc_pinned", i32, [vp, sz, P(vp)])
        sig("lthip_free_pinned", None, [vp, vp])
        sig("lthip_copy_h2d", i32, [vp, vp, vp, sz])
        sig("lthip_copy_d2h", i32, [vp, vp, vp, sz])
        sig("lthip_link_copy", i32, [vp, vp, vp, sz])
        sig("lthip_timing_enable", i32, [vp, i32])
        sig("lthip_timing_reset", i32, [vp])
        sig("lthip_timing_get", i32, [vp, i32, P(C.c_double), P(u64)])
        sig("lthip_plan_create", i32, [vp, u32, vp, vp, u32, u32, u32, P(vp)])
        sig("lthip_plan_destroy", None, [vp, vp])
        sig("lthip_plan_resize_single", i32, [vp, vp, u64])
        sig("lthip_plan_chunk_capacity", u64, [vp])
        sig("lthip_plan_slices", u32, [vp])
        sig("lthip_chunk_hash", i32, [vp, vp, vp, vp, vp, vp, vp, P(u64)])
        sig("lthip_chunk_from_buffer", i32, [vp, vp, u64, u32, u32, u32, P(u64)])
        sig("lthip_hash_ranges", i32, [vp, vp, u64, vp, vp, u32, vp])
        sig("lthip_lz4_bound", sz, [sz])
        sig("lthip_lz4_compress_blocks", i32, [vp, vp, u32, vp, vp, vp, vp, vp, vp, i32])
        sig("lthip_lz4_decompress_blocks", i32, [vp, vp, u32, vp, vp, vp, vp, vp, vp])
        sig("lthip_zstd_bound", sz, [sz])
        sig("lthip_zstd_compress_blocks", i32, [vp, vp, u32, vp, vp, vp, vp, vp, vp])
        sig("lthip_zstd_compress_blocks_q", i32, [vp, vp, u32, vp, vp, vp, vp, vp, vp, i32])
        sig("lthip_zstd_quality_of_settings", i32, [u32])
        sig("lthip_zstd_decompress_blocks", i32, [vp, vp, u32, vp, vp, vp, vp, vp, vp])
        sig("lthip_zstd_debug_units", i32, [vp, u64, u64, vp, vp, vp])
        sig("lthip_zstd_last_decode_stats", i32, [vp, vp])
        sig("lthip_debug_reload_env", None, [])
        sig("lthip_debug_fail_alloc", i32, [C.c_int64, C.c_int64])
        sig("lthip_debug_alloc_calls", C.c_int64, [P(C.c_int64)])
        sig("lthip_stored_block_header_size", sz, [u32])
        sig("lthip_write_stored_block_headers", i32, [vp, u32, vp, vp, vp, u32, u32, vp, vp, vp, vp])
        sig("lthip_create_missing_content", i32, [vp, u64, vp, u64, vp, vp, vp, u32, u32, u32, vp, sz, vp])
        sig("lthip_get_existing_store_index", i32, [vp, vp, sz, u64, vp, u32, vp, sz, vp])
        sig("lthip_version_index_size", sz, [u32, u64, u64, u32])
        sig("lthip_build_version_index", i32, [vp, u32, vp, vp, vp, vp, u32, vp, u64, vp, vp, vp, u32, u32, vp, sz, vp])
        sig("lthip_dedup_first_seen", i32, [vp, u64, vp, vp, vp])
        sig("lthip_dedup_min_ordinal", i32, [vp, u64, vp, vp, vp, vp])
        sig("lthip_ingest_set_first_seen", i32, [vp, vp, u64])
        sig("lthip_plan_reaim", i32, [vp, vp, u32, vp, vp])
        sig("lthip_hash_one", i32, [vp, vp, u32, vp])
        sig("lthip_hash_runs_u64", i32, [vp, vp, vp, u32, vp])
        sig("lthip_hash_runs_u64_bounded", i32, [vp, vp, vp, u32, u64, u64, vp])
        sig("lthip_b3_stream_batch", i32, [vp, vp, u64, vp])
        sig("lthip_b3_stream_final", i32, [vp, vp, u32, u64, vp, vp])
        for name, stream in (("lthip_blake2s", "lthip_b2s_stream"), ("lthip_meow", "lthip_meow_stream")):
            sig(name + "_ranges", i32, [vp, vp, u64, vp, vp, u32, vp])
            sig(name + "_ranges_dev", i32, [vp, vp, u64, vp, vp, vp, u32, vp])
            sig(name + "_one", i32, [vp, vp, u32, vp])
            sig(name + "_runs_u64", i32, [vp, vp, vp, u32, vp])
            sig(name + "_runs_u64_bounded", i32, [vp, vp, vp, u32, u64, u64, vp])
            sig(stream + "_batch", i32, [vp, vp, u64, vp])
            sig(stream + "_final", i32, [vp, vp, u32, u64, vp, vp])
        sig("lthip_dedup_first_seen_range", i32, [vp, u64, vp, u64, u64, vp, vp])
        sig("lthip_gather_ranges", i32, [vp, vp, u64, vp, vp, vp, vp])
        sig("lthip_pack_blocks", i32, [u64, vp, u32, u32, vp, u64, P(u64)])
        sig("lthip_pack_blocks_batch", i32, [u64, vp, u64, u32, u32, u64, u64, u32, u32, vp, vp, u64, P(u64), P(u64)])
        sig("lthip_synth_fill", i32, [vp, vp, u32, vp, vp, vp, i32])
        sig("lthip_synth_fill_ranges", i32, [vp, vp, u32, vp, vp, vp, vp, i32])
        sig("lthip_ingest_create", i32, [vp, vp, P(vp)])
        sig("lthip_ingest_destroy", None, [vp])
        sig("lthip_ingest_index", i32, [vp, vp, vp, vp, u64, vp, vp, u64, vp, sz])
        sig("lthip_ingest_write", i32, [vp, vp, vp, u64])
        sig("lthip_ingest_finish", i32, [vp, vp, sz, vp])
        sig("lthip_ingest_compressed_sizes", vp, [vp])
        sig("lthip_ingest_images", i32, [vp, P(u64), P(u64), P(vp), P(vp)])
        sig("lthip_divtest_eval", i32, [u32, u32])
        sig("lthip_job_count", u64, [u32, vp, u32])
        sig("lthip_make_jobs", i32, [u32, vp, u32, u64, vp, vp, vp])
        sig("lthip_partition_jobs", i32, [u64, vp, u32, i32, vp, vp])
        sig("lthip_exchange_layout", i32, [u64, vp, u32, vp, u64, u64, vp, vp, vp])
        sig("lthip_exchange_ranges", u64, [u64, vp, vp, vp, u64, u64, vp, vp, vp])
        sig("lthip_exchange_reorder", i32, [vp, vp, vp, u32, u64, vp, vp, vp])
        sig("lthip_job_ordinals", i32, [vp, u64, vp, vp, u64, vp])
        sig("lthip_comm_unique_id", i32, [vp])
        sig("lthip_comm_create", i32, [vp, i32, i32, vp, P(vp)])
        sig("lthip_comm_destroy", i32, [vp])
        sig("lthip_comm_allgather", i32, [vp, vp, vp, vp, u64, u32])
        sig("lthip_comm_alltoallv", i32, [vp, vp, vp, vp, vp, vp, vp, vp, u32])
        sig("lthip_comm_info", i32, [vp, P(i32), P(i32), P(i32)])

    def device_count(self) -> int:
        return int(self.dll.lthip_device_count())

    def build_id(self) -> str:
        return self.dll.lthip_build_id().decode()


_lib: Optional[HipLib] = None


ABLATIONS_LIB_PATH = Path(__file__).resolve().parent.parent / "build" / "ablations" / "liblongtail_hip.so"
_abl = None


def load_ablations() -> HipLib:
    global _abl
    if _abl is None:
        if os.environ.get("LTHIP_LIB_PATH"):
            _abl = load()
        else:
            if not ABLATIONS_LIB_PATH.exists():
                raise FileNotFoundError(f"{ABLATIONS_LIB_PATH} is missing: run `make ablations` (or __graft_entry__.build())")
            _abl = HipLib(ABLATIONS_LIB_PATH)
    return _abl


def load(path: Optional[os.PathLike] = None) -> HipLib:
    global _lib
    if _lib is None or path is not None:
        _lib = HipLib(path)
    return _lib


def _ptr(t) -> int:
    if t is None:
        return 0
    if isinstance(t, np.ndarray):
        return t.ctypes.data
    return int(t.data_ptr())


class Context:

    def __init__(self, device: int = 0, stream: "object | None" = "torch", lib: Optional[HipLib] = None):
        import torch

        self.lib = lib or load()
        self.torch = torch
        self.device = device
        if stream == "torch":
            raw_stream = int(torch.cuda.current_stream(device).cuda_stream)
        elif stream is None:
            raw_stream = -1
        else:
            raw_stream = int(stream)
        h = C.c_void_p()
        err = self.lib.dll.lthip_ctx_create(device, C.c_void_p(raw_stream), C.byref(h))
        if err:
            raise LongtailHipError(err, "lthip_ctx_create", "(no GPU?)" if err == errno.ENODEV else "")
        self.h = h

    def close(self):
        if getattr(self, "h", None):
            self.lib.dll.lthip_ctx_destroy(self.h)
            self.h = None

    def __del__(self):
        try:
            self.close()
        except Exception:
            pass

    def _check(self, err: int, what: str):
        if err:
            msg = self.lib.dll.lthip_ctx_error(self.h)
            raise LongtailHipError(err, what, msg.decode() if msg else "")

    def sync(self):
        self._check(self.lib.dll.lthip_ctx_sync(self.h), "lthip_ctx_sync")

    def timing(self, on: bool):
        self._check(self.lib.dll.lthip_timing_enable(self.h, 1 if on else 0), "lthip_timing_enable")

    def timing_reset(self):
        self._check(self.lib.dll.lthip_timing_reset(self.h), "lthip_timing_reset")

    def timing_get(self) -> dict:
        out = {}
        for name, kid in KERNEL_IDS.items():
            ms, n = C.c_double(0), C.c_uint64(0)
            self._check(self.lib.dll.lthip_timing_get(self.h, kid, C.byref(ms), C.byref(n)), "lthip_timing_get")
            out[name] = (ms.value, n.value)
        return out

    def _dev(self):
        return self.torch.device("cuda", self.device)

    def synth_fill(self, dst, offsets, sizes, seeds, kind: int, skips=None):
        o, s, sd = _u64arr(offsets), _u64arr(sizes), _u64arr(seeds)
        sk = _u64arr(skips) if skips is not None else None
        self._check(
            self.lib.dll.lthip_synth_fill_ranges(self.h, _ptr(dst), len(o), o.ctypes.data, s.ctypes.data, sd.ctypes.data,
                                                 sk.ctypes.data if sk is not None else None, kind),
            "lthip_synth_fill_ranges",
        )

    def make_plan(self, part_offsets, part_sizes, min_chunk: int, avg_chunk: int, max_chunk: int) -> "Plan":
        return Plan(self, part_offsets, part_sizes, min_chunk, avg_chunk, max_chunk)

    def chunk_hash(self, plan: "Plan", data, want_hashes: bool = True, outputs=None, sync: bool = True):
        torch = self.torch
        cap = max(1, plan.capacity)
        if outputs is None:
            dev = self._dev()
            offs = torch.empty(cap, dtype=torch.int64, device=dev)
            lens = torch.empty(cap, dtype=torch.int32, device=dev)
            hashes = torch.empty(cap, dtype=torch.int64, device=dev) if want_hashes else None
            first = torch.empty(plan.nparts + 1, dtype=torch.int32, device=dev)
        else:
            offs, lens, hashes, first = outputs
        total = C.c_uint64(0)
        err = self.lib.dll.lthip_chunk_hash(
            self.h, plan.h, _ptr(data), _ptr(offs), _ptr(lens), _ptr(hashes), _ptr(first), C.byref(total) if sync else None
        )
        self._check(err, "lthip_chunk_hash")
        return (int(total.value) if sync else None), offs, lens, hashes, first

    def hash_ranges(self, data, offsets, lens, max_len: int = 0, out=None):
        torch = self.torch
        n = int(offsets.numel())
        if out is None:
            out = torch.empty(max(1, n), dtype=torch.int64, device=self._dev())
        self._check(
            self.lib.dll.lthip_hash_ranges(self.h, _ptr(data), n, _ptr(offsets), _ptr(lens), max_len, _ptr(out)),
            "lthip_hash_ranges",
        )
        return out[:n]

    def _chain_ranges(self, name, data, offsets, lens, max_len, out, count_bound, d_count):
        torch = self.torch
        n = int(offsets.numel()) if count_bound is None else int(count_bound)
        if out is None:
            out = torch.empty(max(1, n), dtype=torch.int64, device=self._dev())
        if d_count is None:
            err = getattr(self.lib.dll, name + "_ranges")(self.h, _ptr(data), n, _ptr(offsets), _ptr(lens), max_len, _ptr(out))
        else:
            err = getattr(self.lib.dll, name + "_ranges_dev")(self.h, _ptr(data), n, _ptr(d_count), _ptr(offsets), _ptr(lens), max_len, _ptr(out))
        self._check(err, name + "_ranges")
        return out[:n]

    def _chain_one(self, name, data, length, out) -> None:
        self._check(getattr(self.lib.dll, name + "_one")(self.h, _ptr(data), length, _ptr(out)), name + "_one")

    def _chain_runs_u64(self, name, values, first, run_count, out):
        if out is None:
            out = self.torch.empty(max(1, run_count), dtype=self.torch.int64, device=self._dev())
        self._check(getattr(self.lib.dll, name + "_runs_u64")(self.h, _ptr(values), _ptr(first), run_count, _ptr(out)), name + "_runs_u64")
        return out[:run_count]

    def _chain_stream(self, name, batch_bytes, state_bytes, data, length) -> int:
        torch = self.torch
        state = torch.empty(state_bytes, dtype=torch.uint8, device=self._dev())
        out = torch.zeros(1, dtype=torch.int64, device=self._dev())
        base = _ptr(data)
        batches = max(0, (length - 1) // batch_bytes)
        for b in range(batches):
            self._check(getattr(self.lib.dll, name + "_batch")(self.h, base + b * batch_bytes, b, _ptr(state)), name + "_batch")
        tail = length - batches * batch_bytes
        self._check(getattr(self.lib.dll, name + "_final")(self.h, base + batches * batch_bytes if tail else None, tail, batches, _ptr(state),
                                                           _ptr(out)), name + "_final")
        return int(out.cpu().numpy().view(np.uint64)[0])

    def blake2s_ranges(self, data, offsets, lens, max_len: int = 0, out=None, count_bound: Optional[int] = None, d_count=None):
        return self._chain_ranges("lthip_blake2s", data, offsets, lens, max_len, out, count_bound, d_count)

    def blake2s_one(self, data, length: int, out) -> None:
        self._chain_one("lthip_blake2s", data, length, out)

    def blake2s_runs_u64(self, values, first, run_count: int, out=None):
        return self._chain_runs_u64("lthip_blake2s", values, first, run_count, out)

    def b2s_stream(self, data, length: int) -> int:
        return self._chain_stream("lthip_b2s_stream", B2S_STREAM_BATCH, B2S_STREAM_STATE_BYTES, data, length)

    def meow_ranges(self, data, offsets, lens, max_len: int = 0, out=None, count_bound: Optional[int] = None, d_count=None):
        return self._chain_ranges("lthip_meow", data, offsets, lens, max_len, out, count_bound, d_count)

    def meow_one(self, data, length: int, out) -> None:
        self._chain_one("lthip_meow", data, length, out)

    def meow_runs_u64(self, values, first, run_count: int, out=None):
        return self._chain_runs_u64("lthip_meow", values, first, run_count, out)

    def meow_stream(self, data, length: int) -> int:
        return self._chain_stream("lthip_meow_stream", MEOW_STREAM_BATCH, MEOW_STREAM_STATE_BYTES, data, length)

    def timing_get_blake2s(self):
        ms, n = C.c_double(0), C.c_uint64(0)
        self._check(self.lib.dll.lthip_timing_get(self.h, BLAKE2S_KERNEL_ID, C.byref(ms), C.byref(n)), "lthip_timing_get")
        return ms.value, n.value

    def chunk_from_buffer(self, data, size: int, min_chunk: int, avg_chunk: int, max_chunk: int) -> int:
        out = C.c_uint64(0)
        self._check(
            self.lib.dll.lthip_chunk_from_buffer(self.h, _ptr(data), size, min_chunk, avg_chunk, max_chunk, C.byref(out)),
            "lthip_chunk_from_buffer",
        )
        return int(out.value)

    def _codec(self, fn, src, src_offsets, src_sizes, dst, dst_offsets, dst_caps, extra=()):
        torch = self.torch
        so, ss = _u64arr(src_offsets), _u32arr(src_sizes)
        do, dc = _u64arr(dst_offsets), _u32arr(dst_caps)
        n = len(so)
        out_sizes = torch.empty(max(1, n), dtype=torch.int32, device=self._dev())
        err = fn(self.h, _ptr(src), n, so.ctypes.data, ss.ctypes.data, _ptr(dst), do.ctypes.data, dc.ctypes.data,
                 _ptr(out_sizes), *extra)
        self._check(err, fn.__name__)
        return out_sizes[:n]

    def lz4_compress_blocks(self, src, src_offsets, src_sizes, dst, dst_offsets, dst_caps, segment_log2: int = 0):
        return self._codec(self.lib.dll.lthip_lz4_compress_blocks, src, src_offsets, src_sizes, dst, dst_offsets,
                           dst_caps, (segment_log2,))

    def lz4_decompress_blocks(self, src, src_offsets, src_sizes, dst, dst_offsets, dst_caps):
        return self._codec(self.lib.dll.lthip_lz4_decompress_blocks, src, src_offsets, src_sizes, dst, dst_offsets,
                           dst_caps)

    def zstd_compress_blocks(self, src, src_offsets, src_sizes, dst, dst_offsets, dst_caps, quality: int = 0):
        return self._codec(self.lib.dll.lthip_zstd_compress_blocks_q, src, src_offsets, src_sizes, dst, dst_offsets,
                           dst_caps, (int(quality),))

    def zstd_decompress_blocks(self, src, src_offsets, src_sizes, dst, dst_offsets, dst_caps):
        return self._codec(self.lib.dll.lthip_zstd_decompress_blocks, src, src_offsets, src_sizes, dst, dst_offsets,
                           dst_caps)

    def zstd_last_decode_stats(self):
        out = np.zeros(4, np.uint32)
        self._check(self.lib.dll.lthip_zstd_last_decode_stats(self.h, out.ctypes.data), "lthip_zstd_last_decode_stats")
        return tuple(int(v) for v in out)

    def zstd_debug_units(self, first: int, count: int):
        meta = np.zeros((count, 4), np.uint32)
        lits = np.zeros((count, 4096), np.uint8)
        recs = np.zeros((count, 1024), np.uint64)
        self._check(self.lib.dll.lthip_zstd_debug_units(self.h, first, count, meta.ctypes.data, lits.ctypes.data,
                                                        recs.ctypes.data), "lthip_zstd_debug_units")
        return meta, lits, recs

    def build_version_index(self, asset_sizes, path_start_offsets, permissions, path_data: bytes, asset_chunk_counts,
                            chunk_hashes, chunk_lens, chunk_total: int, target_chunk_size: int, asset_tags=None,
                            hash_identifier: int = 0x626C6B33) -> bytes:
        n = len(asset_sizes)
        a_sz, a_off = _u64arr(asset_sizes), _u32arr(path_start_offsets)
        a_perm = np.ascontiguousarray(np.asarray(permissions, dtype=np.uint16))
        a_cnt = _u32arr(asset_chunk_counts)
        a_tag = _u32arr(asset_tags) if asset_tags is not None else None
        cap = self.lib.dll.lthip_version_index_size(n, chunk_total, chunk_total, len(path_data))
        out = np.zeros(cap + 16, np.uint8)
        size = C.c_size_t(0)
        err = self.lib.dll.lthip_build_version_index(
            self.h, n, a_sz.ctypes.data, a_off.ctypes.data, a_perm.ctypes.data, path_data, len(path_data), a_cnt.ctypes.data,
            chunk_total, _ptr(chunk_hashes), _ptr(chunk_lens), a_tag.ctypes.data if a_tag is not None else None, hash_identifier,
            target_chunk_size, out.ctypes.data, cap, C.byref(size))
        self._check(err, "lthip_build_version_index")
        return out[: size.value].tobytes()

    def write_stored_block_headers(self, block_first_chunk, chunk_hashes, chunk_lens, tag: int, raw_sizes, comp_sizes, arena,
                                   image_offsets, hash_identifier: int = 0x626C6B33):
        bf, rs, io = _u64arr(block_first_chunk), _u32arr(raw_sizes), _u64arr(image_offsets)
        self._check(self.lib.dll.lthip_write_stored_block_headers(self.h, len(io), bf.ctypes.data, _ptr(chunk_hashes), _ptr(chunk_lens),
                                                                  hash_identifier, tag, rs.ctypes.data, _ptr(comp_sizes), _ptr(arena),
                                                                  io.ctypes.data), "lthip_write_stored_block_headers")

    def create_missing_content(self, existing_hashes, chunk_hashes, chunk_lens, chunk_tags, max_block_size: int,
                               max_chunks_per_block: int, hash_identifier: int = 0x626C6B33) -> bytes:
        ne = int(existing_hashes.numel()) if existing_hashes is not None else 0
        n = int(chunk_hashes.numel())
        tags = _u32arr(chunk_tags) if chunk_tags is not None else None
        cap = 16 + 20 * n + 12 * n + 64
        out = np.zeros(cap, np.uint8)
        size = C.c_size_t(0)
        err = self.lib.dll.lthip_create_missing_content(
            self.h, ne, _ptr(existing_hashes) if ne else None, n, _ptr(chunk_hashes), _ptr(chunk_lens),
            tags.ctypes.data if tags is not None else None, hash_identifier, max_block_size, max_chunks_per_block, out.ctypes.data,
            cap, C.byref(size))
        self._check(err, "lthip_create_missing_content")
        return out[: size.value].tobytes()

    def get_existing_store_index(self, store_index: bytes, chunk_hashes, min_block_usage_percent: int) -> bytes:
        raw = np.frombuffer(store_index, np.uint8)
        n = int(chunk_hashes.numel()) if chunk_hashes is not None else 0
        out = np.zeros(len(raw) + 64, np.uint8)
        size = C.c_size_t(0)
        err = self.lib.dll.lthip_get_existing_store_index(self.h, raw.ctypes.data, len(raw), n, _ptr(chunk_hashes) if n else None,
                                                          min_block_usage_percent, out.ctypes.data, len(out), C.byref(size))
        self._check(err, "lthip_get_existing_store_index")
        return out[: size.value].tobytes()

    def link_copy(self, dst, src, nbytes: int):
        self._check(self.lib.dll.lthip_link_copy(self.h, _ptr(dst), _ptr(src), nbytes), "lthip_link_copy")

    def gather_ranges(self, src, src_offsets, lens, dst, dst_offsets):
        n = int(src_offsets.numel())
        self._check(self.lib.dll.lthip_gather_ranges(self.h, _ptr(src), n, _ptr(src_offsets), _ptr(lens), _ptr(dst),
                                                     _ptr(dst_offsets)), "lthip_gather_ranges")

    def exchange_reorder(self, gathered, out, ranges):
        r_src, r_dst, r_cnt = ranges
        assert gathered.dtype == out.dtype and gathered.is_contiguous() and out.is_contiguous()
        self._check(self.lib.dll.lthip_exchange_reorder(self.h, _ptr(gathered), _ptr(out), gathered.element_size(), len(r_src),
                                                        r_src.ctypes.data, r_dst.ctypes.data, r_cnt.ctypes.data), "lthip_exchange_reorder")

    def job_ordinals(self, local_first: np.ndarray, global_first: np.ndarray, local_chunks: int):
        lf, gf = _u32arr(local_first), _u32arr(global_first)
        assert len(lf) == len(gf)
        out = self.torch.empty(max(1, local_chunks), dtype=self.torch.int32, device=self._dev())
        self._check(self.lib.dll.lthip_job_ordinals(self.h, len(lf), lf.ctypes.data, gf.ctypes.data, local_chunks, _ptr(out)),
                    "lthip_job_ordinals")
        return out[:local_chunks]

    def dedup_first_seen_range(self, hashes, first: int, count: int):
        torch = self.torch
        n = int(hashes.numel())
        out = torch.empty(max(1, count), dtype=torch.int32, device=self._dev())
        uniq = torch.zeros(1, dtype=torch.int64, device=self._dev())
        self._check(self.lib.dll.lthip_dedup_first_seen_range(self.h, n, _ptr(hashes), first, count, _ptr(out), _ptr(uniq)),
                    "lthip_dedup_first_seen_range")
        return out[:count], uniq

    def dedup_first_seen(self, hashes):
        torch = self.torch
        n = int(hashes.numel())
        first = torch.empty(max(1, n), dtype=torch.int32, device=self._dev())
        uniq = torch.zeros(1, dtype=torch.int64, device=self._dev())
        self._check(self.lib.dll.lthip_dedup_first_seen(self.h, n, _ptr(hashes), _ptr(first), _ptr(uniq)),
                    "lthip_dedup_first_seen")
        return first[:n], uniq

    def dedup_min_ordinal(self, hashes, ordinals, sync: bool = True):
        torch = self.torch
        n = int(hashes.numel())
        first = torch.empty(max(1, n), dtype=torch.int32, device=self._dev())
        uniq = torch.zeros(1, dtype=torch.int64, device=self._dev())
        self._check(self.lib.dll.lthip_dedup_min_ordinal(self.h, n, _ptr(hashes.contiguous()), _ptr(ordinals.contiguous()), _ptr(first), _ptr(uniq)),
                    "lthip_dedup_min_ordinal")
        if not sync:
            return first[:n], uniq
        self.sync()
        return first[:n], int(uniq.item())


class Comm:

    ID_BYTES = 128
    TRANSPORTS = {1: "rccl", 2: "host-shm"}

    @staticmethod
    def unique_id(lib: Optional[HipLib] = None) -> bytes:
        lib = lib or load()
        buf = (C.c_ubyte * Comm.ID_BYTES)()
        err = lib.dll.lthip_comm_unique_id(C.addressof(buf))
        if err:
            raise LongtailHipError(err, "lthip_comm_unique_id")
        return bytes(buf)

    def __init__(self, ctx: "Optional[Context]", nranks: int, rank: int, unique_id: bytes, lib: Optional[HipLib] = None):
        assert len(unique_id) == Comm.ID_BYTES
        self.ctx, self.nranks, self.rank = ctx, nranks, rank
        self.lib = ctx.lib if ctx is not None else (lib or load())
        buf = (C.c_ubyte * Comm.ID_BYTES).from_buffer_copy(unique_id)
        h = C.c_void_p()
        self._check(self.lib.dll.lthip_comm_create(self._ctx_h(), nranks, rank, C.addressof(buf), C.byref(h)), "lthip_comm_create")
        self.h = h

    def _ctx_h(self):
        return self.ctx.h if self.ctx is not None else None

    def _check(self, err, what):
        if self.ctx is not None:
            self.ctx._check(err, what)
        elif err:
            raise LongtailHipError(err, what)

    def sync(self):
        if self.ctx is not None:
            self.ctx.sync()

    def info(self) -> dict:
        n, r, t = C.c_int32(), C.c_int32(), C.c_int32()
        self._check(self.lib.dll.lthip_comm_info(self.h, C.byref(n), C.byref(r), C.byref(t)), "lthip_comm_info")
        return {"nranks": int(n.value), "rank": int(r.value), "transport": Comm.TRANSPORTS.get(int(t.value), str(t.value))}

    def allgather(self, send, recv=None):
        import torch

        send = send.contiguous()
        if recv is None:
            recv = torch.empty(send.numel() * self.nranks, dtype=send.dtype, device=send.device)
        self._check(self.lib.dll.lthip_comm_allgather(self._ctx_h(), self.h, _ptr(send), _ptr(recv), send.numel(), send.element_size()),
                    "lthip_comm_allgather")
        return recv

    def alltoallv(self, send, send_counts, recv_counts, recv=None):
        import torch

        send = send.contiguous()
        sc = np.ascontiguousarray(send_counts, dtype=np.uint64)
        rc = np.ascontiguousarray(recv_counts, dtype=np.uint64)
        assert len(sc) == self.nranks and len(rc) == self.nranks and int(sc.sum()) == send.numel()
        sd = np.zeros(self.nranks, np.uint64)
        rd = np.zeros(self.nranks, np.uint64)
        np.cumsum(sc[:-1], out=sd[1:])
        np.cumsum(rc[:-1], out=rd[1:])
        if recv is None:
            recv = torch.empty(int(rc.sum()), dtype=send.dtype, device=send.device)
        self._check(self.lib.dll.lthip_comm_alltoallv(self._ctx_h(), self.h, _ptr(send) if send.numel() else None, sc.ctypes.data, sd.ctypes.data,
                                                      _ptr(recv) if recv.numel() else None, rc.ctypes.data, rd.ctypes.data, send.element_size()),
                    "lthip_comm_alltoallv")
        return recv

    def close(self):
        if self.h:
            self.lib.dll.lthip_comm_destroy(self.h)
            self.h = None


class IngestConfig(C.Structure):
    _fields_ = [("target_chunk_size", C.c_uint32), ("hash_identifier", C.c_uint32), ("max_block_size", C.c_uint32),
                ("max_chunks_per_block", C.c_uint32), ("compression_type", C.c_uint32), ("codec", C.c_uint32),
                ("batch_bytes", C.c_uint64)]


class IngestTree(C.Structure):
    _fields_ = [("asset_count", C.c_uint32), ("asset_sizes", C.c_void_p), ("path_start_offsets", C.c_void_p),
                ("permissions", C.c_void_p), ("path_data", C.c_char_p), ("path_data_size", C.c_uint32), ("asset_tags", C.c_void_p),
                ("job_count", C.c_uint64), ("job_asset", C.c_void_p), ("job_first", C.c_void_p), ("my_job_count", C.c_uint64),
                ("my_jobs", C.c_void_p)]


class IngestResult(C.Structure):
    _fields_ = [(n, C.c_uint64) for n in ("struct_size", "chunks_all", "unique_all", "chunks_local", "unique_local", "blocks", "raw_bytes",
                                          "compressed_bytes", "gathered_blocks", "version_index_size", "store_index_size", "gathered_bytes")]


CODECS = {"none": 0, "lz4": 1, "zstd": 2}
LZ4_TYPE = 0x6C7A3432
ZSTD_DEFAULT = 0x7A746432


class Ingest:

    def __init__(self, ctx: "Context", target_chunk_size: int, max_block_size: int, max_chunks_per_block: int, codec: str,
                 compression_type: Optional[int] = None, batch_bytes: int = 0, hash_identifier: int = 0x626C6B33):
        self.ctx = ctx
        if compression_type is None:
            compression_type = LZ4_TYPE if codec == "lz4" else ZSTD_DEFAULT
        self.cfg = IngestConfig(target_chunk_size, hash_identifier, max_block_size, max_chunks_per_block, compression_type,
                                CODECS[codec], batch_bytes)
        h = C.c_void_p()
        ctx._check(ctx.lib.dll.lthip_ingest_create(ctx.h, C.byref(self.cfg), C.byref(h)), "lthip_ingest_create")
        self.h = h
        self._keep = None

    def close(self):
        if getattr(self, "h", None):
            self.ctx.lib.dll.lthip_ingest_destroy(self.h)
            self.h = None

    def __del__(self):
        try:
            self.close()
        except Exception:
            pass

    @staticmethod
    def tree(asset_sizes, path_start_offsets, permissions, path_data: bytes, job_asset, job_first, my_jobs=None, asset_tags=None):
        a_sz, a_off = _u64arr(asset_sizes), _u32arr(path_start_offsets)
        a_perm = np.ascontiguousarray(np.asarray(permissions, dtype=np.uint16))
        j_as, j_first = _u32arr(job_asset), _u64arr(job_first)
        mine = _u64arr(my_jobs) if my_jobs is not None else None
        tags = _u32arr(asset_tags) if asset_tags is not None else None
        t = IngestTree(len(a_sz), a_sz.ctypes.data, a_off.ctypes.data, a_perm.ctypes.data, path_data, len(path_data),
                       tags.ctypes.data if tags is not None else None, len(j_as), j_as.ctypes.data, j_first.ctypes.data,
                       len(mine) if mine is not None else 0, mine.ctypes.data if mine is not None else None)
        keep = [a_sz, a_off, a_perm, path_data, j_as, j_first, mine, tags]
        t._keep = keep
        return t, keep

    def index(self, tree: IngestTree, all_hashes, all_lens, all_chunks: int, local_offsets, local_part_first, local_chunks: int,
              version_index_out=None):
        cap = 0 if version_index_out is None else (version_index_out.numel() if hasattr(version_index_out, "numel") else len(version_index_out))
        err = self.ctx.lib.dll.lthip_ingest_index(self.h, C.byref(tree), _ptr(all_hashes), _ptr(all_lens), all_chunks, _ptr(local_offsets),
                                                  _ptr(local_part_first), local_chunks, _ptr(version_index_out) or None, cap)
        self._index_keep = (tree, all_hashes, all_lens, local_offsets, local_part_first, version_index_out)
        self.ctx._check(err, "lthip_ingest_index")

    def set_first_seen(self, first_index, unique_chunks: int):
        self._first_keep = first_index
        self.ctx._check(self.ctx.lib.dll.lthip_ingest_set_first_seen(self.h, _ptr(first_index), C.c_uint64(int(unique_chunks))),
                        "lthip_ingest_set_first_seen")

    def write(self, data, arena):
        self.ctx._check(self.ctx.lib.dll.lthip_ingest_write(self.h, _ptr(data), _ptr(arena), int(arena.numel())), "lthip_ingest_write")

    def finish(self, store_index_out=None) -> IngestResult:
        cap = 0 if store_index_out is None else (store_index_out.numel() if hasattr(store_index_out, "numel") else len(store_index_out))
        res = IngestResult()
        res.struct_size = C.sizeof(IngestResult)
        err = self.ctx.lib.dll.lthip_ingest_finish(self.h, _ptr(store_index_out) or None, cap, C.byref(res))
        self.ctx._check(err, "lthip_ingest_finish")
        self._index_keep = None
        return res

    def images(self):
        first, count, po, ps = C.c_uint64(), C.c_uint64(), C.c_void_p(), C.c_void_p()
        self.ctx._check(self.ctx.lib.dll.lthip_ingest_images(self.h, C.byref(first), C.byref(count), C.byref(po), C.byref(ps)), "lthip_ingest_images")
        n = int(count.value)
        if n == 0:
            return int(first.value), np.zeros(0, np.uint64), np.zeros(0, np.uint32)
        return (int(first.value), np.ctypeslib.as_array((C.c_uint64 * n).from_address(po.value)).copy(),
                np.ctypeslib.as_array((C.c_uint32 * n).from_address(ps.value)).copy())

    def compressed_sizes(self, nblocks: int) -> np.ndarray:
        p = self.ctx.lib.dll.lthip_ingest_compressed_sizes(self.h)
        if not p or nblocks == 0:
            return np.zeros(0, np.uint32)
        return np.ctypeslib.as_array((C.c_uint32 * nblocks).from_address(p)).copy()


class Plan:
    def __init__(self, ctx: Context, part_offsets, part_sizes, min_chunk: int, avg_chunk: int, max_chunk: int):
        self.ctx = ctx
        o, s = _u64arr(part_offsets), _u64arr(part_sizes)
        assert len(o) == len(s)
        self.nparts = len(o)
        h = C.c_void_p()
        err = ctx.lib.dll.lthip_plan_create(ctx.h, self.nparts, o.ctypes.data, s.ctypes.data, min_chunk, avg_chunk,
                                            max_chunk, C.byref(h))
        ctx._check(err, "lthip_plan_create")
        self.h = h
        self.capacity = int(ctx.lib.dll.lthip_plan_chunk_capacity(h))
        self.total_bytes = int(s.sum()) if len(s) else 0

    @property
    def slices(self) -> int:
        return int(self.ctx.lib.dll.lthip_plan_slices(self.h))

    def reaim(self, part_offsets, part_sizes):
        o, s = _u64arr(part_offsets), _u64arr(part_sizes)
        assert len(o) == len(s)
        self.ctx._check(self.ctx.lib.dll.lthip_plan_reaim(self.ctx.h, self.h, len(o), o.ctypes.data, s.ctypes.data), "lthip_plan_reaim")
        self.nparts = len(o)
        self.capacity = int(self.ctx.lib.dll.lthip_plan_chunk_capacity(self.h))
        self.total_bytes = int(s.sum()) if len(s) else 0

    def close(self):
        if getattr(self, "h", None) and getattr(self.ctx, "h", None):
            self.ctx.lib.dll.lthip_plan_destroy(self.ctx.h, self.h)
        self.h = None

    def __del__(self):
        try:
            self.close()
        except Exception:
            pass


def pack_blocks(lens: np.ndarray, max_block_size: int, max_chunks_per_block: int, lib: Optional[HipLib] = None) -> np.ndarray:
    lib = lib or load()
    lens = np.ascontiguousarray(lens, dtype=np.uint32)
    cap = len(lens) + 2
    starts = np.zeros(cap, dtype=np.uint64)
    nb = C.c_uint64(0)
    err = lib.dll.lthip_pack_blocks(len(lens), lens.ctypes.data, max_block_size, max_chunks_per_block, starts.ctypes.data, cap,
                                    C.byref(nb))
    if err:
        raise LongtailHipError(err, "lthip_pack_blocks")
    return starts[: nb.value + 1].astype(np.int64)


class BatchPacker:

    def __init__(self, lens: np.ndarray, max_block_size: int, max_chunks_per_block: int, max_batch_bytes: int, arena_bytes: int,
                 bound_div: int, bound_add: int, lib: Optional[HipLib] = None):
        self.lib = lib or load()
        self.lens = np.ascontiguousarray(lens, dtype=np.uint32)
        self.args = (max_block_size, max_chunks_per_block, max_batch_bytes, arena_bytes, bound_div, bound_add)
        self.pos = 0
        self.cap = int(min(len(self.lens), max_batch_bytes // max(1, max_block_size // 2) + len(self.lens) // max_chunks_per_block + 8) + 2)
        self.starts = np.empty(self.cap, dtype=np.uint64)
        self.sizes = np.empty(self.cap, dtype=np.uint64)

    def next(self):
        if self.pos >= len(self.lens):
            return None
        nb, nxt = C.c_uint64(0), C.c_uint64(0)
        mb, mc, bb, ab, bd, ba = self.args
        err = self.lib.dll.lthip_pack_blocks_batch(len(self.lens), self.lens.ctypes.data, self.pos, mb, mc, bb, ab, bd, ba,
                                                   self.starts.ctypes.data, self.sizes.ctypes.data, self.cap, C.byref(nb), C.byref(nxt))
        if err:
            raise LongtailHipError(err, "lthip_pack_blocks_batch")
        self.pos = nxt.value
        n = nb.value
        return self.starts[: n + 1].astype(np.int64), self.sizes[:n].astype(np.int64)


def chunker_params(target_chunk_size: int, chunker_min: int = 48):
    mn = max(chunker_min, target_chunk_size // 8)
    av = max(chunker_min, target_chunk_size // 2)
    mx = max(chunker_min, target_chunk_size * 2)
    return mn, av, mx
```

Measured before the change: 841.8.

## Add per-part walking buzhash kernel that scans only cut-candidate tiles

Adds a new chunking kernel in which each wave takes a whole part from an atomic ticket and walks its chunk boundaries sequentially. It DMAs and evaluates only the tiles between min_chunk and max_chunk of the current chunk, optionally prefetching the guessed next tile. This skips the bytes below min_chunk and removes the bitmap write plus the separate select pass. A plan flag, driven by the part count per resident wave and the maximum part size, picks walk or bitmap scan per slice, and the DMA helpers are moved into a shared struct. The trade-off is serial per-part work that can load-imbalance when parts are few or large.

```diff
diff --git a/include/longtail_hip.h b/include/longtail_hip.h
--- a/include/longtail_hip.h
+++ b/include/longtail_hip.h
@@ -94,6 +94,7 @@
 LTHIP_EXPORT void lthip_plan_destroy(lthip_ctx* ctx, lthip_plan* plan);
 LTHIP_EXPORT uint64_t lthip_plan_chunk_capacity(const lthip_plan* plan);
 LTHIP_EXPORT uint32_t lthip_plan_slices(const lthip_plan* plan);
+LTHIP_EXPORT uint32_t lthip_plan_walked_scans(const lthip_plan* plan);
 
 LTHIP_EXPORT int lthip_chunk_hash(lthip_ctx* ctx, const lthip_plan* plan, const void* d_data, uint64_t* d_chunk_offsets,
                                   uint32_t* d_chunk_lens, uint64_t* d_chunk_hashes, uint32_t* d_part_first,
@@ -195,6 +196,7 @@
 LTHIP_EXPORT void lthip_debug_reload_env(void);
 LTHIP_EXPORT int lthip_debug_fail_alloc(int64_t after, int64_t count);
 LTHIP_EXPORT int64_t lthip_debug_alloc_calls(int64_t* out_failed);
+LTHIP_EXPORT int lthip_debug_walk_tiles(uint64_t* out_tiles);
 LTHIP_EXPORT int lthip_zstd_debug_units(lthip_ctx* ctx, uint64_t first, uint64_t count, void* h_meta, void* h_lits,
                                         void* h_recs);
 
diff --git a/longtail_amd/csrc/k_buzhash.hip b/longtail_amd/csrc/k_buzhash.hip
--- a/longtail_amd/csrc/k_buzhash.hip
+++ b/longtail_amd/csrc/k_buzhash.hip
@@ -269,53 +269,74 @@
 
 constexpr int DMA_BUF_B = WROWS * 64;
 
-template <int MODE, int WAVES>
-__global__ __launch_bounds__(64 * WAVES, 1) void k_buzhash_prefix_dma(const uint8_t* __restrict__ data,
-                                                                       const PartDev* __restrict__ parts,
-                                                                       const uint32_t* __restrict__ tile_part,
-                                                                       uint32_t ntiles, DivTest dv,
-                                                                       uint64_t* __restrict__ bm0,
-                                                                       uint64_t* __restrict__ bm1)
-{
-    extern __shared__ __attribute__((aligned(16))) uint32_t smem[];
-    const int tid = threadIdx.x;
-    const int lane = tid & 63;
-    const int wave = __builtin_amdgcn_readfirstlane(tid >> 6);
-    uint32_t* buf = smem + 256 * TAB_REP + wave * ((DMA_BUF_B >> 2) + HALO_DW);
-    uint32_t* halo = buf + (DMA_BUF_B >> 2);
-    prefix_table_init(smem, tid, 64 * WAVES);
-
-    const uint32_t buf_byte = __builtin_amdgcn_readfirstlane((uint32_t)(uintptr_t)(const __attribute__((address_space(3))) uint32_t*)buf);
-    PrefixConsts pc;
-    pc.lane4 = (uint32_t)lane * 4u;
-    pc.hj = 63u - (uint32_t)lane;
-    pc.halo_byte = buf_byte + DMA_BUF_B;
-    pc.thr = MODE == 1 ? 0u : 0xFFFFFFFFu / (dv.d >> dv.k2);
-    pc.exact_add = dv.addc - dv.inv;
-
-    const uint32_t src_vec = 4u * ((uint32_t)lane >> 2) + (((uint32_t)lane & 3u) ^ (((uint32_t)lane >> 4) & 3u));
-    const uint32_t src_off = 16u * src_vec;
-    const uint32_t own_f = (((uint32_t)lane + 1u) >> 2) & 3u;
-    const uint32_t own_row = buf_byte + 64u * ((uint32_t)lane + 1u);
-
-    const uint64_t nwt = (uint64_t)ntiles * 4u;
-    const uint64_t wstride = (uint64_t)gridDim.x * (uint64_t)WAVES;
-    uint64_t wt = (uint64_t)blockIdx.x * (uint64_t)WAVES + (uint64_t)wave;
-    if (wt >= nwt)
-        return;
-
-    const uint32_t buf_mid = buf_byte + 2048u;
-    auto piece = [&](auto U, const uint8_t* mid_src) __attribute__((always_inline))
-    {
-        constexpr int u = decltype(U)::value;
-        const uint32_t so = src_off, bm = buf_mid;
+struct TileDma
+{
+    const uint8_t* data;
+    uint32_t* buf;
+    int lane;
+    uint32_t buf_byte;
+    uint32_t buf_mid;
+    uint32_t src_off;
+    uint32_t own_row;
+    uint32_t own_f;
+
+    __device__ __forceinline__ TileDma(const uint8_t* d, uint32_t* b, int ln) : data(d), buf(b), lane(ln)
+    {
+        buf_byte = __builtin_amdgcn_readfirstlane((uint32_t)(uintptr_t)(const __attribute__((address_space(3))) uint32_t*)buf);
+        buf_mid = buf_byte + 2048u;
+        const uint32_t src_vec = 4u * ((uint32_t)lane >> 2) + (((uint32_t)lane & 3u) ^ (((uint32_t)lane >> 4) & 3u));
+        src_off = 16u * src_vec;
+        own_f = (((uint32_t)lane + 1u) >> 2) & 3u;
+        own_row = buf_byte + 64u * ((uint32_t)lane + 1u);
+    }
+
+    template <int MODE>
+    __device__ __forceinline__ PrefixConsts consts(const DivTest& dv) const
+    {
+        PrefixConsts pc;
+        pc.lane4 = (uint32_t)lane * 4u;
+        pc.hj = 63u - (uint32_t)lane;
+        pc.halo_byte = buf_byte + DMA_BUF_B;
+        pc.thr = MODE == 1 ? 0u : 0xFFFFFFFFu / (dv.d >> dv.k2);
+        pc.exact_add = dv.addc - dv.inv;
+        return pc;
+    }
+
+    template <int u>
+    __device__ __forceinline__ void piece(const uint8_t* mid_src) const
+    {
         asm volatile("s_mov_b32 m0, %[l]\n\ts_nop 0\n\t"
                      "global_load_lds_dwordx4 %[v], %[b] offset:%[o]"
                      :
-                     : [v] "v"(so), [l] "s"(bm), [b] "s"(mid_src), [o] "i"(1024 * u - 2048)
+                     : [v] "v"(src_off), [l] "s"(buf_mid), [b] "s"(mid_src), [o] "i"(1024 * u - 2048)
                      : "memory");
-    };
-    auto issue = [&](const PartDev& p, uint64_t sp) __attribute__((always_inline))
+    }
+
+    template <int u>
+    __device__ __forceinline__ void edge(const PartDev& p, uint64_t sp, const uint8_t* mid_src) const
+    {
+        const int64_t g = (int64_t)sp - 64 + 1024 * u + (int64_t)src_off;
+        const bool lane_on = u < 4 || lane < 4;
+        const bool whole = lane_on && g >= 0 && (uint64_t)g + 16 <= p.size;
+        const bool part = lane_on && g >= 0 && (uint64_t)g < p.size && (uint64_t)g + 16 > p.size;
+        if (whole)
+            piece<u>(mid_src);
+        if (part)
+        {
+            const uint8_t* src = data + p.off;
+            uint32_t w[4] = {0, 0, 0, 0};
+            const uint32_t n = (uint32_t)(p.size - (uint64_t)g);
+            for (uint32_t bb = 0; bb < n; ++bb)
+                w[bb >> 2] |= (uint32_t)src[g + bb] << (8 * (bb & 3));
+            uint32_t* d = buf + 256 * u + 4 * lane;
+            d[0] = w[0];
+            d[1] = w[1];
+            d[2] = w[2];
+            d[3] = w[3];
+        }
+    }
+
+    __device__ __forceinline__ void issue(const PartDev& p, uint64_t sp) const
     {
         const uint8_t* mid_src = data + p.off + sp - 64 + 2048;
         if (sp >= 64 && sp + (uint64_t)WTILE <= p.size)
@@ -329,51 +350,21 @@
                          : [v] "v"(src_off), [l] "s"(buf_mid), [b] "s"(mid_src)
                          : "memory");
             if (lane < 4)
-                piece(std::integral_constant<int, 4>{}, mid_src);
+                piece<4>(mid_src);
         }
         else
         {
-            auto edge = [&](auto U) __attribute__((always_inline))
-            {
-                constexpr int u = decltype(U)::value;
-                const int64_t g = (int64_t)sp - 64 + 1024 * u + (int64_t)src_off;
-                const bool lane_on = u < 4 || lane < 4;
-                const bool whole = lane_on && g >= 0 && (uint64_t)g + 16 <= p.size;
-                const bool part = lane_on && g >= 0 && (uint64_t)g < p.size && (uint64_t)g + 16 > p.size;
-                if (whole)
-                    piece(U, mid_src);
-                if (part)
-                {
-                    const uint8_t* src = data + p.off;
-                    uint32_t w[4] = {0, 0, 0, 0};
-                    const uint32_t n = (uint32_t)(p.size - (uint64_t)g);
-                    for (uint32_t bb = 0; bb < n; ++bb)
-                        w[bb >> 2] |= (uint32_t)src[g + bb] << (8 * (bb & 3));
-                    uint32_t* d = buf + 256 * u + 4 * lane;
-                    d[0] = w[0];
-                    d[1] = w[1];
-                    d[2] = w[2];
-                    d[3] = w[3];
-                }
-            };
-            edge(std::integral_constant<int, 0>{});
-            edge(std::integral_constant<int, 1>{});
-            edge(std::integral_constant<int, 2>{});
-            edge(std::integral_constant<int, 3>{});
-            edge(std::integral_constant<int, 4>{});
-        }
-    };
-
-    PartDev pd = parts[tile_part[wt >> 2]];
-    uint64_t span = ((wt >> 2) - pd.tile_base) * (uint64_t)TILE + (wt & 3u) * (uint64_t)WTILE;
-    issue(pd, span);
-
-    uint64_t pend_m = 0, pend_summary = 0, pend_i0 = 0, pend_i1 = 0;
-    bool pend = false;
-    for (;;)
+            edge<0>(p, sp, mid_src);
+            edge<1>(p, sp, mid_src);
+            edge<2>(p, sp, mid_src);
+            edge<3>(p, sp, mid_src);
+            edge<4>(p, sp, mid_src);
+        }
+    }
+
+    __device__ __forceinline__ void take(uint32_t (&win)[16], uint32_t& hb, const PrefixConsts& pc) const
     {
         asm volatile("s_waitcnt vmcnt(0)" ::: "memory");
-        uint32_t win[16];
 #pragma unroll
         for (int c = 0; c < 4; ++c)
         {
@@ -383,8 +374,46 @@
             win[4 * c + 2] = q.z;
             win[4 * c + 3] = q.w;
         }
-        const uint32_t hb = lds_load_u8(buf_byte + pc.hj);
+        hb = lds_load_u8(buf_byte + pc.hj);
         asm volatile("s_waitcnt lgkmcnt(0)" ::: "memory");
+    }
+};
+
+template <int MODE, int WAVES>
+__global__ __launch_bounds__(64 * WAVES, 1) void k_buzhash_prefix_dma(const uint8_t* __restrict__ data,
+                                                                       const PartDev* __restrict__ parts,
+                                                                       const uint32_t* __restrict__ tile_part,
+                                                                       uint32_t ntiles, DivTest dv,
+                                                                       uint64_t* __restrict__ bm0,
+                                                                       uint64_t* __restrict__ bm1)
+{
+    extern __shared__ __attribute__((aligned(16))) uint32_t smem[];
+    const int tid = threadIdx.x;
+    const int lane = tid & 63;
+    const int wave = __builtin_amdgcn_readfirstlane(tid >> 6);
+    uint32_t* buf = smem + 256 * TAB_REP + wave * ((DMA_BUF_B >> 2) + HALO_DW);
+    uint32_t* halo = buf + (DMA_BUF_B >> 2);
+    prefix_table_init(smem, tid, 64 * WAVES);
+
+    const TileDma dma(data, buf, lane);
+    const PrefixConsts pc = dma.consts<MODE>(dv);
+
+    const uint64_t nwt = (uint64_t)ntiles * 4u;
+    const uint64_t wstride = (uint64_t)gridDim.x * (uint64_t)WAVES;
+    uint64_t wt = (uint64_t)blockIdx.x * (uint64_t)WAVES + (uint64_t)wave;
+    if (wt >= nwt)
+        return;
+
+    PartDev pd = parts[tile_part[wt >> 2]];
+    uint64_t span = ((wt >> 2) - pd.tile_base) * (uint64_t)TILE + (wt & 3u) * (uint64_t)WTILE;
+    dma.issue(pd, span);
+
+    uint64_t pend_m = 0, pend_summary = 0, pend_i0 = 0, pend_i1 = 0;
+    bool pend = false;
+    for (;;)
+    {
+        uint32_t win[16], hb;
+        dma.take(win, hb, pc);
 
         if (pend)
         {
@@ -401,7 +430,7 @@
         {
             npd = parts[tile_part[next >> 2]];
             next_span = ((next >> 2) - npd.tile_base) * (uint64_t)TILE + (next & 3u) * (uint64_t)WTILE;
-            issue(npd, next_span);
+            dma.issue(npd, next_span);
         }
 
         pend_m = prefix_legal(prefix_tile<MODE>(win, hb, pc, dv, lane, halo), span + (uint64_t)lane * RUN, pd.size);
@@ -511,6 +540,159 @@
         part_count[p] = n;
 }
 
+#ifdef LTHIP_ABLATIONS
+__device__ unsigned long long g_walk_tiles;
+#endif
+
+template <int MODE, int WAVES, bool GUESS>
+__global__ __launch_bounds__(64 * WAVES, 1) void k_buzhash_walk(const uint8_t* __restrict__ data, const PartDev* __restrict__ parts,
+                                                                 uint32_t nparts, DivTest dv, uint32_t min_chunk, uint32_t max_chunk,
+                                                                 uint2* __restrict__ region, uint32_t* __restrict__ part_count,
+                                                                 uint32_t* __restrict__ ticket)
+{
+    extern __shared__ __attribute__((aligned(16))) uint32_t smem[];
+    const int tid = threadIdx.x;
+    const int lane = tid & 63;
+    const int wave = __builtin_amdgcn_readfirstlane(tid >> 6);
+    uint32_t* buf = smem + 256 * TAB_REP + wave * ((DMA_BUF_B >> 2) + HALO_DW);
+    uint32_t* halo = buf + (DMA_BUF_B >> 2);
+    prefix_table_init(smem, tid, 64 * WAVES);
+
+    const TileDma dma(data, buf, lane);
+    const PrefixConsts pc = dma.consts<MODE>(dv);
+    const int lane_base = lane * RUN;
+
+    auto jump = [](uint64_t q) __attribute__((always_inline)) { return q >= 64 ? ((q - 64) & ~(uint64_t)15) + 64 : (uint64_t)0; };
+
+    bool inflight = false;
+    uint64_t inflight_tb = 0;
+#ifdef LTHIP_ABLATIONS
+    uint32_t tiles = 0;
+#endif
+    for (;;)
+    {
+        __builtin_amdgcn_wave_barrier();
+        uint32_t t = atomicAdd(ticket, lane == 0 ? 1u : 0u);
+        t = __builtin_amdgcn_readfirstlane(t);
+        if (t >= nparts)
+            break;
+        const PartDev pd = parts[t];
+        const uint64_t size = pd.size;
+        uint2* out = region + pd.region_base;
+        uint64_t s = 0, qlo = 0, qhi = 0;
+        uint32_t n = 0, end = 0;
+
+        auto next_chunk = [&]() __attribute__((always_inline)) -> bool
+        {
+            for (;;)
+            {
+                if (s >= size)
+                    return false;
+                const uint64_t left = size - s;
+                const uint32_t len = left <= min_chunk ? (uint32_t)left : left > max_chunk ? max_chunk : (uint32_t)left;
+                if (left > min_chunk && len > min_chunk)
+                {
+                    end = len;
+                    qlo = s + min_chunk;
+                    qhi = s + end - 1;
+                    return true;
+                }
+                if (lane == 0)
+                    out[n] = make_uint2((uint32_t)s, len);
+                ++n;
+                s += len;
+            }
+        };
+
+        if (next_chunk())
+        {
+            uint64_t tb = jump(qlo);
+            for (bool walking = true; walking;)
+            {
+                if (!(inflight && inflight_tb == tb))
+                {
+                    if (inflight)
+                        asm volatile("s_waitcnt vmcnt(0)" ::: "memory");
+                    dma.issue(pd, tb);
+                }
+                inflight = false;
+                uint32_t win[16], hb;
+                dma.take(win, hb, pc);
+                if (GUESS)
+                {
+                    uint64_t g = tb + (uint64_t)WTILE;
+                    bool aim = true;
+                    if (g > qhi)
+                    {
+                        const uint64_t s2 = s + end;
+                        aim = size - s2 > min_chunk && max_chunk > min_chunk;
+                        g = jump(s2 + min_chunk);
+                    }
+                    if (aim)
+                    {
+                        dma.issue(pd, g);
+                        inflight = true;
+                        inflight_tb = g;
+                    }
+                }
+                const uint64_t raw = prefix_tile<MODE>(win, hb, pc, dv, lane, halo);
+#ifdef LTHIP_ABLATIONS
+                ++tiles;
+#endif
+                for (;;)
+                {
+                    const int lo = (int)(qlo > tb ? qlo - tb : 0) - lane_base;
+                    const int hi = (int)(qhi - tb < (uint64_t)WTILE ? qhi - tb : (uint64_t)WTILE - 1) - lane_base;
+                    uint64_t m = raw;
+                    if (lo > 0)
+                        m = lo > 63 ? 0ull : m & (~0ull << lo);
+                    if (hi < 63)
+                        m = hi < 0 ? 0ull : m & ((2ull << hi) - 1ull);
+                    const uint64_t any = __builtin_amdgcn_ballot_w64(m != 0ull);
+                    uint32_t len;
+                    if (any != 0ull)
+                    {
+                        const int f = __builtin_ctzll(any);
+                        const uint64_t q = tb + (uint64_t)(f * RUN + __builtin_ctzll(bcast64(m, f)));
+                        len = (uint32_t)(q - s) + 1u;
+                    }
+                    else if (qhi - tb < (uint64_t)WTILE)
+                        len = end;
+                    else
+                    {
+                        tb += (uint64_t)WTILE;
+                        break;
+                    }
+                    if (lane == 0)
+                        out[n] = make_uint2((uint32_t)s, len);
+                    ++n;
+                    s += len;
+                    if (!next_chunk())
+                    {
+                        walking = false;
+                        break;
+                    }
+                    if (qlo >= tb && qlo - tb < (uint64_t)WTILE)
+                        continue;
+                    tb = jump(qlo);
+                    break;
+                }
+            }
+        }
+        if (inflight)
+        {
+            asm volatile("s_waitcnt vmcnt(0)" ::: "memory");
+            inflight = false;
+        }
+        if (lane == 0)
+            part_count[t] = n;
+    }
+#ifdef LTHIP_ABLATIONS
+    if (lane == 0 && tiles)
+        atomicAdd(&g_walk_tiles, (unsigned long long)tiles);
+#endif
+}
+
 constexpr int SCAN_THREADS = 256;
 constexpr int SCAN_ITEMS = 8;
 constexpr int SCAN_BLOCK = SCAN_THREADS * SCAN_ITEMS;
@@ -800,6 +982,82 @@
         return launch_buzhash_roll(ctx, plan, d_data, bm0, bm1);
 #endif
     return launch_buzhash_prefix<16, true>(ctx, plan, d_data, bm0, bm1);
+}
+
+uint32_t lthip_k1_resident_waves(int device)
+{
+    static std::atomic<uint32_t> cached[64] = {};
+    if (device >= 0 && device < 64 && cached[device].load(std::memory_order_relaxed))
+        return cached[device].load(std::memory_order_relaxed);
+    int ncu = 256;
+    (void)hipDeviceGetAttribute(&ncu, hipDeviceAttributeMultiprocessorCount, device);
+    const uint32_t w = (uint32_t)(ncu > 0 ? ncu : 256) * 16u;
+    if (device >= 0 && device < 64)
+        cached[device].store(w, std::memory_order_relaxed);
+    return w;
+}
+
+#ifndef K1_WALK_GUESS
+#define K1_WALK_GUESS 1
+#endif
+
+template <bool GUESS>
+static int launch_buzhash_walk(lthip_ctx* ctx, const lthip_plan* plan, const uint8_t* d_data, uint2* region, uint32_t* part_count)
+{
+    constexpr int WAVES = 16;
+    const size_t lds = sizeof(uint32_t) * (256 * TAB_REP + WAVES * ((DMA_BUF_B >> 2) + HALO_DW));
+    auto k0 = &k_buzhash_walk<0, WAVES, GUESS>;
+    auto k1 = &k_buzhash_walk<1, WAVES, GUESS>;
+    static bool granted[64] = {};
+    if (ctx->device < 0 || ctx->device >= 64 || !granted[ctx->device])
+    {
+        LTHIP_CHECK(ctx, hipFuncSetAttribute(reinterpret_cast<const void*>(k0), hipFuncAttributeMaxDynamicSharedMemorySize, (int)lds));
+        LTHIP_CHECK(ctx, hipFuncSetAttribute(reinterpret_cast<const void*>(k1), hipFuncAttributeMaxDynamicSharedMemorySize, (int)lds));
+        if (ctx->device >= 0 && ctx->device < 64)
+            granted[ctx->device] = true;
+    }
+    void* ticket;
+    int err = lthip_scratch(ctx, S_WALK_TICKET, 64, &ticket);
+    if (err)
+        return err;
+    uint32_t grid = lthip_k1_resident_waves(ctx->device) / WAVES;
+    if ((uint64_t)grid * WAVES > plan->nparts)
+        grid = (uint32_t)div_up_u64(plan->nparts, WAVES);
+    LaunchTimer t(ctx, LTHIP_K_BUZHASH);
+    LTHIP_CHECK(ctx, hipMemsetAsync(ticket, 0, 4, ctx->stream));
+    hipLaunchKernelGGL(plan->div.pow2 ? k1 : k0, dim3(grid), dim3(64 * WAVES), lds, ctx->stream, d_data, plan->d_parts, plan->nparts,
+                       plan->div, plan->min_chunk, plan->max_chunk, region, part_count, (uint32_t*)ticket);
+    LTHIP_LAUNCH_CHECK(ctx);
+    return 0;
+}
+
+int lthip_launch_buzhash_walk(lthip_ctx* ctx, const lthip_plan* plan, const uint8_t* d_data, uint2* region, uint32_t* part_count)
+{
+    if (plan->nparts == 0)
+        return 0;
+#ifdef LTHIP_ABLATIONS
+    LTHIP_ABLATION_ENV(env_guess, "LTHIP_K1_WALK_GUESS");
+    if (env_guess.get() >= 0 && (env_guess.get() != 0) != (K1_WALK_GUESS != 0))
+        return launch_buzhash_walk<!K1_WALK_GUESS>(ctx, plan, d_data, region, part_count);
+#endif
+    return launch_buzhash_walk<K1_WALK_GUESS != 0>(ctx, plan, d_data, region, part_count);
+}
+
+extern "C" int lthip_debug_walk_tiles(uint64_t* out_tiles)
+{
+#ifdef LTHIP_ABLATIONS
+    if (!out_tiles)
+        return EINVAL;
+    unsigned long long v = 0, zero = 0;
+    if (hipDeviceSynchronize() != hipSuccess || hipMemcpyFromSymbol(&v, HIP_SYMBOL(g_walk_tiles), sizeof v) != hipSuccess ||
+        hipMemcpyToSymbol(HIP_SYMBOL(g_walk_tiles), &zero, sizeof zero) != hipSuccess)
+        return EIO;
+    *out_tiles = v;
+    return 0;
+#else
+    (void)out_tiles;
+    return ENOTSUP;
+#endif
 }
 
 int lthip_launch_select(lthip_ctx* ctx, const lthip_plan* plan, const uint64_t* bm0, const uint64_t* bm1, uint2* region,
diff --git a/longtail_amd/csrc/lthip_ctx.hip b/longtail_amd/csrc/lthip_ctx.hip
--- a/longtail_amd/csrc/lthip_ctx.hip
+++ b/longtail_amd/csrc/lthip_ctx.hip
@@ -608,8 +608,17 @@
         x.chunk_cap += cap;
         x.total_bytes += sz;
         x.leaf_cap += div_up_u64(sz, 1024) + cap;
-    }
-    return 0;
+        x.nonempty_parts += sz != 0;
+        x.max_part_bytes = sz > x.max_part_bytes ? sz : x.max_part_bytes;
+    }
+    return 0;
+}
+
+static bool plan_walk_rule(const lthip_plan* plan)
+{
+    const uint64_t waves = lthip_k1_resident_waves(plan->device);
+    return plan->nonempty_parts >= LTHIP_WALK_MIN_PARTS_PER_WAVE * waves &&
+           plan->max_part_bytes * LTHIP_WALK_MAX_PART_DIV <= plan->total_bytes / waves;
 }
 
 static int plan_create_impl(lthip_ctx* ctx, uint32_t part_count, const uint64_t* part_offsets, const uint64_t* part_sizes,
@@ -645,6 +654,7 @@
     plan->capacity_bytes = x.total_bytes;
     plan->cap_parts = part_count ? part_count : 1;
     plan->cap_tiles = x.ntiles ? x.ntiles : 1;
+    plan->walked = plan_walk_rule(plan);
 
     hipError_t e = lthip_hip_malloc((void**)&plan->d_parts, sizeof(PartDev) * plan->cap_parts);
     if (e == hipSuccess)
@@ -670,6 +680,7 @@
 static int plan_aim(lthip_ctx* ctx, lthip_plan* plan, const PlanExtents& x, const PartDev* parts)
 {
     static_cast<PlanExtents&>(*plan) = x;
+    plan->walked = plan_walk_rule(plan);
     const int err = lthip_stage_upload(ctx, plan->d_parts, parts, sizeof(PartDev) * x.nparts, ctx->stream);
     return err ? err : lthip_launch_tile_table(ctx, plan);
 }
@@ -793,28 +804,58 @@
 extern "C" uint64_t lthip_plan_chunk_capacity(const lthip_plan* plan) { return plan ? plan->chunk_cap : 0; }
 extern "C" uint32_t lthip_plan_slices(const lthip_plan* plan) { return plan && plan->sliced ? plan->nslices : 1u; }
 
-static int chunk_bitmaps(lthip_ctx* ctx, const lthip_plan* plan, uint64_t** bm0, uint64_t** bm1)
-{
-    const int err = lthip_scratch(ctx, S_BM0, plan->bm0_words * 8, (void**)bm0);
-    return err ? err : lthip_scratch(ctx, S_BM1, plan->bm1_words * 8, (void**)bm1);
-}
-
-static int chunk_scan(lthip_ctx* ctx, const lthip_plan* plan, const void* d_data, uint64_t* bm0, uint64_t* bm1)
-{
-    return plan->nparts ? lthip_launch_buzhash(ctx, plan, (const uint8_t*)d_data, bm0, bm1) : 0;
-}
-
-static int chunk_cut_hash(lthip_ctx* ctx, const lthip_plan* plan, const void* d_data, const uint64_t* bm0, const uint64_t* bm1,
-                          uint64_t* d_offsets, uint32_t* d_lens, uint64_t* d_hashes, uint32_t* d_part_first)
-{
-    void *region, *pcount;
+static bool plan_walks(const lthip_plan* plan)
+{
+    LTHIP_ABLATION_ENV(env_walk, "LTHIP_K1_WALK");
+    if (env_walk.get() >= 0)
+        return env_walk.get() != 0 && plan->nparts != 0;
+    return plan->walked;
+}
+extern "C" uint32_t lthip_plan_walked_scans(const lthip_plan* plan)
+{
+    if (!plan)
+        return 0;
+    if (!plan->sliced)
+        return plan_walks(plan);
+    uint32_t n = 0;
+    for (uint32_t k = 0; k < plan->nslices; ++k)
+        n += plan_walks(plan->slice[k]);
+    return n;
+}
+
+struct ScanBuffers
+{
+    uint64_t *bm0, *bm1;
+    uint2* region;
+    uint32_t* part_count;
+};
+static int chunk_scan_buffers(lthip_ctx* ctx, const lthip_plan* plan, bool bitmaps, ScanBuffers* b)
+{
+    b->bm0 = b->bm1 = nullptr;
     int err;
-    if ((err = lthip_scratch(ctx, S_REGION, plan->chunk_cap * sizeof(uint2), &region)) ||
-        (err = lthip_scratch(ctx, S_PART_COUNT, ((size_t)plan->nparts + 1) * 4, &pcount)))
+    if (bitmaps && ((err = lthip_scratch(ctx, S_BM0, plan->bm0_words * 8, (void**)&b->bm0)) ||
+                    (err = lthip_scratch(ctx, S_BM1, plan->bm1_words * 8, (void**)&b->bm1))))
         return err;
-    if (plan->nparts && (err = lthip_launch_select(ctx, plan, bm0, bm1, (uint2*)region, (uint32_t*)pcount)))
+    if ((err = lthip_scratch(ctx, S_REGION, plan->chunk_cap * sizeof(uint2), (void**)&b->region)))
         return err;
-    if ((err = lthip_launch_compact(ctx, plan, (const uint2*)region, (const uint32_t*)pcount, d_part_first, d_offsets, d_lens)))
+    return lthip_scratch(ctx, S_PART_COUNT, ((size_t)plan->nparts + 1) * 4, (void**)&b->part_count);
+}
+
+static int chunk_scan(lthip_ctx* ctx, const lthip_plan* plan, const void* d_data, const ScanBuffers& b)
+{
+    if (!plan->nparts)
+        return 0;
+    return plan_walks(plan) ? lthip_launch_buzhash_walk(ctx, plan, (const uint8_t*)d_data, b.region, b.part_count)
+                            : lthip_launch_buzhash(ctx, plan, (const uint8_t*)d_data, b.bm0, b.bm1);
+}
+
+static int chunk_cut_hash(lthip_ctx* ctx, const lthip_plan* plan, const void* d_data, const ScanBuffers& b, uint64_t* d_offsets,
+                          uint32_t* d_lens, uint64_t* d_hashes, uint32_t* d_part_first)
+{
+    int err;
+    if (plan->nparts && !plan_walks(plan) && (err = lthip_launch_select(ctx, plan, b.bm0, b.bm1, b.region, b.part_count)))
+        return err;
+    if ((err = lthip_launch_compact(ctx, plan, b.region, b.part_count, d_part_first, d_offsets, d_lens)))
         return err;
     return d_hashes ? lthip_launch_blake3(ctx, (const uint8_t*)d_data, d_offsets, d_lens, d_part_first + plan->nparts, plan->chunk_cap,
                                           plan->leaf_cap, plan->max_chunk, d_hashes)
@@ -854,10 +895,11 @@
         parts_rest += (uint64_t)plan->slice[k]->nparts + 1;
     }
     void *x_off, *x_len, *x_hash, *x_first;
-    uint64_t *bm0, *bm1;
+    ScanBuffers sb;
+    const bool bitmaps = lthip_plan_walked_scans(plan) != S;
     if (lthip_scratch(ctx, S_SLICE_OFFS, cap_rest * 8, &x_off) || lthip_scratch(ctx, S_SLICE_LENS, cap_rest * 4, &x_len) ||
         lthip_scratch(ctx, S_SLICE_HASH, cap_rest * 8, &x_hash) || lthip_scratch(ctx, S_SLICE_FIRST, parts_rest * 4, &x_first) ||
-        chunk_bitmaps(ctx, plan, &bm0, &bm1))
+        chunk_scan_buffers(ctx, plan, bitmaps, &sb))
     {
         ctx->err[0] = 0;
         return 0;
@@ -878,7 +920,7 @@
         first_k[k] = k ? (uint32_t*)x_first + po : d_part_first;
         co += k ? pk->chunk_cap + 1 : 0;
         po += k ? (uint64_t)pk->nparts + 1 : 0;
-        if ((err = chunk_scan(ctx, pk, d_data, bm0, bm1)))
+        if ((err = chunk_scan(ctx, pk, d_data, sb)))
             break;
         hipEvent_t scanned = lthip_sync_event(ctx);
         hipError_t e = hipEventRecord(scanned, ctx->stream);
@@ -886,10 +928,15 @@
             e = hipStreamWaitEvent(c2->stream, scanned, 0);
         if (e != hipSuccess)
             err = lthip_fail(ctx, EIO, "lthip_chunk_hash (the wait of the second stream for a scan)", hipGetErrorString(e));
-        else if ((err = chunk_cut_hash(c2, pk, d_data, bm0, bm1, offs_k[k], lens_k[k], hash_k[k], first_k[k])))
+        else if ((err = chunk_cut_hash(c2, pk, d_data, sb, offs_k[k], lens_k[k], hash_k[k], first_k[k])))
             (void)lthip_fail(ctx, err, "lthip_chunk_hash (a slice on the second stream)", c2->err);
-        bm0 += pk->bm0_words;
-        bm1 += pk->bm1_words;
+        if (bitmaps)
+        {
+            sb.bm0 += pk->bm0_words;
+            sb.bm1 += pk->bm1_words;
+        }
+        sb.region += pk->chunk_cap;
+        sb.part_count += pk->nparts;
     }
     hipEvent_t hashed = lthip_sync_event(ctx);
     hipError_t e = hipEventRecord(hashed, c2->stream);
@@ -927,9 +974,9 @@
     LTHIP_CHECK(ctx, hipSetDevice(ctx->device));
     bool sliced;
     int err = chunk_hash_sliced(ctx, plan, d_data, d_chunk_offsets, d_chunk_lens, d_chunk_hashes, d_part_first, &sliced);
-    uint64_t *bm0, *bm1;
-    if (!sliced && !(err = chunk_bitmaps(ctx, plan, &bm0, &bm1)) && !(err = chunk_scan(ctx, plan, d_data, bm0, bm1)))
-        err = chunk_cut_hash(ctx, plan, d_data, bm0, bm1, d_chunk_offsets, d_chunk_lens, d_chunk_hashes, d_part_first);
+    ScanBuffers sb;
+    if (!sliced && !(err = chunk_scan_buffers(ctx, plan, !plan_walks(plan), &sb)) && !(err = chunk_scan(ctx, plan, d_data, sb)))
+        err = chunk_cut_hash(ctx, plan, d_data, sb, d_chunk_offsets, d_chunk_lens, d_chunk_hashes, d_part_first);
     if (err)
         return err;
     if (out_total)
diff --git a/longtail_amd/csrc/lthip_internal.h b/longtail_amd/csrc/lthip_internal.h
--- a/longtail_amd/csrc/lthip_internal.h
+++ b/longtail_amd/csrc/lthip_internal.h
@@ -43,6 +43,8 @@
     uint64_t bm0_words;
     uint64_t bm1_words;
     uint64_t leaf_cap;
+    uint32_t nonempty_parts;
+    uint64_t max_part_bytes;
 };
 
 struct lthip_plan : PlanExtents
@@ -59,7 +61,10 @@
     uint32_t slice_first[9];
     uint32_t nslices;
     bool sliced;
-};
+    bool walked;
+};
+constexpr uint32_t LTHIP_WALK_MIN_PARTS_PER_WAVE = 2;
+constexpr uint32_t LTHIP_WALK_MAX_PART_DIV = 2;
 constexpr uint64_t LTHIP_SLICE_MIN_BYTES = 1ull << 30;
 #ifndef LTHIP_SLICES
 #define LTHIP_SLICES 2
@@ -101,6 +106,7 @@
     S_SLICE_HASH,
     S_SLICE_FIRST,
     S_LEN_CLASS_ORDER,
+    S_WALK_TICKET,
     S_COUNT
 };
 
@@ -219,6 +225,8 @@
 
 int lthip_launch_tile_table(lthip_ctx* ctx, lthip_plan* plan);
 int lthip_launch_buzhash(lthip_ctx* ctx, const lthip_plan* plan, const uint8_t* d_data, uint64_t* bm0, uint64_t* bm1);
+int lthip_launch_buzhash_walk(lthip_ctx* ctx, const lthip_plan* plan, const uint8_t* d_data, uint2* region, uint32_t* part_count);
+uint32_t lthip_k1_resident_waves(int device);
 int lthip_launch_select(lthip_ctx* ctx, const lthip_plan* plan, const uint64_t* bm0, const uint64_t* bm1, uint2* region,
                         uint32_t* part_count);
 int lthip_launch_compact(lthip_ctx* ctx, const lthip_plan* plan, const uint2* region, const uint32_t* part_count,
diff --git a/longtail_amd/lib.py b/longtail_amd/lib.py
--- a/longtail_amd/lib.py
+++ b/longtail_amd/lib.py
@@ -114,6 +114,7 @@
         sig("lthip_plan_resize_single", i32, [vp, vp, u64])
         sig("lthip_plan_chunk_capacity", u64, [vp])
         sig("lthip_plan_slices", u32, [vp])
+        sig("lthip_plan_walked_scans", u32, [vp])
         sig("lthip_chunk_hash", i32, [vp, vp, vp, vp, vp, vp, vp, P(u64)])
         sig("lthip_chunk_from_buffer", i32, [vp, vp, u64, u32, u32, u32, P(u64)])
         sig("lthip_hash_ranges", i32, [vp, vp, u64, vp, vp, u32, vp])
@@ -130,6 +131,7 @@
         sig("lthip_debug_reload_env", None, [])
         sig("lthip_debug_fail_alloc", i32, [C.c_int64, C.c_int64])
         sig("lthip_debug_alloc_calls", C.c_int64, [P(C.c_int64)])
+        sig("lthip_debug_walk_tiles", i32, [P(C.c_uint64)])
         sig("lthip_stored_block_header_size", sz, [u32])
         sig("lthip_write_stored_block_headers", i32, [vp, u32, vp, vp, vp, u32, u32, vp, vp, vp, vp])
         sig("lthip_create_missing_content", i32, [vp, u64, vp, u64, vp, vp, vp, u32, u32, u32, vp, sz, vp])
@@ -729,6 +731,10 @@
     def slices(self) -> int:
         return int(self.ctx.lib.dll.lthip_plan_slices(self.h))
 
+    @property
+    def walked_scans(self) -> int:
+        return int(self.ctx.lib.dll.lthip_plan_walked_scans(self.h))
+
     def reaim(self, part_offsets, part_sizes):
         o, s = _u64arr(part_offsets), _u64arr(part_sizes)
         assert len(o) == len(s)
```

New measurement: 896.9 (median of 6 runs). 1.07x the previous value.
